# 87003697/DynamiCrafter

Hardware: AMD Instinct MI355X
Metric: frames/sec (and denoising-step ms), 16f@576x1024, DDIM 50 (higher is better)
Workload: dtype bf16; 1 GPU; inference_1024_v1.0.yaml: 1 clip/GPU, 16 frames, latent 72x128, DDIM 50 uniform_trailing eta=1, CFG 7.5 batched (cond+uncond), guidance_rescale 0.7, v-param+ZTSNR+dynamic rescale, hipGraph-captured step; clips_per_gpu=1, parallelism=dp1 over 1 distinct clips (no data-path collective), conditioning=local (1 rank), outputs_finite=True

## Files before the change

### dynamicrafter_amd/_hip.py

```python
import ctypes as C
import os
import threading

_HERE = os.path.dirname(os.path.abspath(__file__))
LIB_PATH = os.environ.get("DC_HIP_LIB") or os.path.join(_HERE, "csrc", "libdcrafter_hip.so")

DC_GEMM_OUT_F32 = 1
DC_GEMM_GEGLU = 2
DC_GEMM_GELU = 4


class DcGemmParams(C.Structure):
    _fields_ = [
        ("A", C.c_void_p), ("W", C.c_void_p), ("C", C.c_void_p), ("bias", C.c_void_p),
        ("rowvec", C.c_void_p), ("residual", C.c_void_p),
        ("lda", C.c_int), ("ldc", C.c_int), ("ldr", C.c_int), ("rowvec_ld", C.c_int),
        ("rows_per_vec", C.c_int),
        ("M", C.c_int), ("N", C.c_int), ("K", C.c_int), ("n_pad", C.c_int),
        ("mode", C.c_int), ("Cin", C.c_int),
        ("IH", C.c_int), ("IW", C.c_int), ("OH", C.c_int), ("OW", C.c_int),
        ("stride", C.c_int), ("pad", C.c_int), ("ups", C.c_int),
        ("T", C.c_int), ("HW", C.c_int),
        ("flags", C.c_int), ("alpha", C.c_float),
        ("workspace", C.c_void_p), ("workspace_bytes", C.c_longlong),
    ]


class DcDdimParams(C.Structure):
    _fields_ = [
        ("a_t", C.c_void_p), ("a_prev", C.c_void_p), ("sigma_t", C.c_void_p), ("sqrt_one_minus_at", C.c_void_p),
        ("sqrt_acp_t", C.c_void_p), ("sqrt_1macp_t", C.c_void_p), ("scale_ratio", C.c_void_p),
        ("step_index", C.c_void_p),
        ("index", C.c_int), ("v_param", C.c_int),
        ("cfg_scale", C.c_float), ("cfg_img", C.c_float), ("guidance_rescale", C.c_float),
        ("temperature", C.c_float),
        ("e_nchw", C.c_int), ("noise_step_stride", C.c_int64),
    ]


class DcDpmParams(C.Structure):
    _fields_ = [
        ("A", C.c_void_p), ("alpha_t", C.c_void_p), ("alpha_p_r", C.c_void_p), ("k", C.c_void_p), ("N", C.c_void_p),
        ("sqrt_one_minus_at", C.c_void_p), ("sqrt_acp_t", C.c_void_p), ("sqrt_1macp_t", C.c_void_p),
        ("scale_ratio", C.c_void_p), ("step_index", C.c_void_p),
        ("index", C.c_int), ("v_param", C.c_int),
        ("cfg_scale", C.c_float), ("cfg_img", C.c_float), ("guidance_rescale", C.c_float),
        ("temperature", C.c_float),
        ("e_nchw", C.c_int), ("noise_step_stride", C.c_int64), ("x0_hist", C.c_void_p),
    ]


class DcSdsParams(C.Structure):
    _fields_ = [
        ("c1", C.c_void_p), ("c2", C.c_void_p), ("w", C.c_void_p), ("step_size", C.c_void_p), ("bc2_sqrt", C.c_void_p),
        ("step_index", C.c_void_p), ("index", C.c_int), ("weight_type", C.c_int), ("x0_param", C.c_int),
        ("e_nchw", C.c_int), ("cfg_scale", C.c_float), ("guidance_rescale", C.c_float),
        ("beta2", C.c_float), ("eps", C.c_float), ("one_minus_beta1", C.c_float), ("one_minus_beta2", C.c_float),
        ("decay", C.c_float), ("grad_scale", C.c_float), ("noise_step_stride", C.c_int64), ("loss", C.c_void_p),
    ]


_P, _I, _F, _L = C.c_void_p, C.c_int, C.c_float, C.c_int64
SIGNATURES = {
    "dc_gemm_conv": (_I, [C.POINTER(DcGemmParams), _P]),
    "dc_gemm_workspace_bytes": (_L, []),
    "dc_gemm_last_variant": (C.c_char_p, []),
    "dc_gemm_set_plan": (_I, [_I]),
    "dc_groupnorm": (_I, [_P, _I, _P, _I, _P, _P, _I, _I, _I, _I, _F, _I, _P, _P]),
    "dc_groupnorm_workspace_bytes": (_L, [_I, _I, _I]),
    "dc_layernorm": (_I, [_P, _I, _P, _I, _P, _P, _I, _I, _F, _P]),
    "dc_flash_attn_d64": (_I, [_P, _P, _P, _P, _I, _I, _I, _I, _I, _I, _I, _I, _L, _L, _F, _I, _F, _P]),
    "dc_ff_geglu_fused320": (_I, [_P, _I, _P, _P, _F, _P, _P, _P, _P, _P, _I, _P, _I, _I, _P]),
    "dc_ff_geglu_proj_fused320": (_I, [_P, _I, _P, _P, _F, _P, _P, _P, _P, _P, _P, _P, _I, _P, _I, _I, _P]),
    "dc_ln_linear": (_I, [_P, _I, _I, _P, _P, _F, _P, _P, _P, _I, _I, _I, _P]),
    "dc_ln_qkv_temporal_attn320": (_I, [_P, _I, _P, _P, _F, _P, _P, _I, _I, _I, _I, _F, _P]),
    "dc_ln_qkv_temporal_attn640": (_I, [_P, _I, _P, _P, _F, _P, _P, _I, _I, _I, _I, _F, _P]),
    "dc_gn_silu_tconv3": (_I, [_P, _I, _I, _P, _P, _P, _I, _P, _P, _P, _I, _P, _I, _I, _I, _I, _I, _P]),
    "dc_groupnorm_stats": (_I, [_P, _I, _I, _I, _I, _I, _F, _P, _P, _P]),
    "dc_gn_linear": (_I, [_P, _I, _I, _P, _P, _P, _I, _I, _P, _P, _P, _I, _I, _I, _P]),
    "dc_flash_attn_set_mode": (_I, [_I, _F]),
    "dc_linear_residual": (_I, [_P, _I, _I, _P, _P, _P, _I, _P, _I, _I, _I, _P]),
    "dc_cross_attn_dual_d64": (_I, [_P, _P, _P, _P, _P, _P, _I, _I, _I, _I, _I, _I, _I, _I, _L, _L, _F, _F, _P]),
    "dc_temporal_attn_d64": (_I, [_P, _I, _P, _I, _I, _I, _I, _I, _F, _P]),
    "dc_gemv_small": (_I, [_P, _I, _P, _P, _P, _I, _I, _I, _I, _I, _I, _I, _P]),
    "dc_timestep_embedding": (_I, [_P, _P, _I, _P, _I, _I, _F, _P]),
    "dc_pack_latent": (_I, [_P, _P, _P, _I, _I, _I, _I, _I, _I, _I, _P]),
    "dc_pack_latent_windows": (_I, [_P, _P, _P, _P, _P] + [_I] * 13 + [_P]),
    "dc_window_merge": (_I, [_P, _I, _P, _I, _P, _P, _P] + [_I] * 12 + [_P]),
    "dc_nchw_to_rows": (_I, [_P, _P, _I, _I, _I, _I, _F, _P]),
    "dc_rows_to_nchw": (_I, [_P, _I, _I, _P, _I, _I, _I, _F, _P]),
    "dc_im2col3x3_c8": (_I, [_P, _I, _P, _I, _I, _I, _I, _P]),
    "dc_copy2d": (_I, [_P, _I, _P, _I, _I, _I, _P]),
    "dc_build_context": (_I, [_P, _P, _I, _I, _I, _I, _I, _P]),
    "dc_softmax_rows": (_I, [_P, _I, _P, _I, _I, _I, _P]),
    "dc_transpose": (_I, [_P, _I, _P, _I, _I, _I, _P]),
    "dc_add_rows": (_I, [_P, _I, _P, _I, _P, _I, _I, _I, _P]),
    "dc_vae_sample": (_I, [_P, _I, _P, _P, _I, _I, _I, _F, _P]),
    "dc_ddim_step": (_I, [C.POINTER(DcDdimParams), _P, _P, _P, _I, _P, _P, _P, _P, _I, _I, _I, _P, _P]),
    "dc_dpmpp_step": (_I, [C.POINTER(DcDpmParams), _P, _P, _P, _I, _P, _P, _P, _P, _I, _I, _I, _P, _P]),
    "dc_sds_noise": (_I, [C.POINTER(DcSdsParams), _P, _P, _P, _I, _L, _P]),
    "dc_sds_step": (_I, [C.POINTER(DcSdsParams), _P, _P, _I, _P, _P, _P, _P, _I, _I, _I, _P, _P]),
    "dc_attn_small": (_I, [_P, _P, _P, _P, _I, _I, _I, _I, _I, _I, _I, _I, _I, _F, _I, _P]),
    "dc_attn_small_lds_bytes": (_L, [_I, _I]),
    "dc_clip_preprocess": (_I, [_P, _P, _P, _P, _I, _I, _I, _I, _I, _I, _I, C.POINTER(_F), C.POINTER(_F), _P]),
    "dc_patchify": (_I, [_P, _P, _I, _I, _I, _I, _I, _I, _P]),
    "dc_embed_tokens": (_I, [_P, _P, _P, _P, _I, _I, _I, _I, _P]),
    "dc_frames_to_u8": (_I, [_P, _P, _I, _I, _I, _I, _I, _P]),
    "dc_jpeg_dct_quant": (_I, [_P, _P, _P, _I, _I, _I, _P]),
    "dc_jpeg_entropy": (_I, [_P, _P, _P, _I, _I, _I, _I, _L, _P]),
    "dc_jpeg_pack": (_I, [_P, _P, _P, _P, _P, _I, _I, _L, _L, _P]),
    "dc_prep_resize_h": (_I, [_P, _P, _P, _P, _P] + [_I] * 8 + [_P]),
    "dc_prep_finish": (_I, [_P, _P, _P, _P, _P] + [_I] * 15 + [_P]),
    "dc_mask_blend": (_I, [_P, _P, _P, _P, _P, _P, _P, _I, _L, _L, _I, _P]),
    "dc_advance_counter": (_I, [_P, _P]),
    "dc_stream_create": (_I, [C.POINTER(_P)]),
    "dc_stream_destroy": (_I, [_P]),
    "dc_stream_sync": (_I, [_P]),
    "dc_graph_begin_capture": (_I, [_P]),
    "dc_graph_end_capture": (_I, [_P, C.POINTER(_P)]),
    "dc_graph_launch": (_I, [_P, _P]),
    "dc_graph_destroy": (_I, [_P]),
    "dc_event_create": (_I, [C.POINTER(_P)]),
    "dc_event_record": (_I, [_P, _P]),
    "dc_event_elapsed_ms": (_I, [_P, _P, C.POINTER(_F)]),
    "dc_event_destroy": (_I, [_P]),
    "dc_error_word_read": (_I, [C.POINTER(C.c_int), _I]),
    "dc_version": (C.c_char_p, []),
}

_lib = None
_lock = threading.Lock()


def lib():
    global _lib
    if _lib is not None:
        return _lib
    with _lock:
        if _lib is None:
            if not os.path.exists(LIB_PATH):
                raise RuntimeError(
                    f"{LIB_PATH} not found: build it with dynamicrafter_amd/csrc/build.sh "
                    "(or __graft_entry__.build()); the HIP extension is mandatory, there is no fallback")
            import torch
            l = C.CDLL(LIB_PATH)
            for name, (res, args) in SIGNATURES.items():
                fn = getattr(l, name)
                fn.restype = res
                fn.argtypes = args
            _lib = l
    return _lib


ERROR_WORD_BITS = {1: "gemm_pipe320x16_kernel: LDS counter wait timed out",
                   2: "flash_attn_d64_pipe_kernel: K/V ring counter wait timed out",
                   4: "gemm_pp_kernel: LDS counter wait timed out"}


def check_error_word(what="", reset=True):
    w = C.c_int(0)
    check(lib().dc_error_word_read(C.byref(w), 1 if reset else 0), "dc_error_word_read")
    if w.value:
        names = [v for k, v in ERROR_WORD_BITS.items() if w.value & k] or [f"unknown bits {w.value:#x}"]
        raise RuntimeError(f"HIP kernels reported a failed wait ({what or 'error word'} = {w.value:#x}): " + "; ".join(names)
                           + " - results since the last check are NOT valid")


def check(code, what):
    if code != 0:
        raise RuntimeError(f"{what} failed with code {code}"
                           + (" (DC_ERR_SHAPE)" if code == -1 else " (DC_ERR_ARG)" if code == -2 else " (hipError_t)"))
```

### dynamicrafter_amd/csrc/dc_common.h

```cpp
#pragma once
#include <hip/hip_runtime.h>
#include <stdint.h>
#include <atomic>

typedef uint16_t bf16_t;

typedef __attribute__((ext_vector_type(8))) short bf16x8_t;
typedef __attribute__((ext_vector_type(4))) short bf16x4_t;
typedef __attribute__((ext_vector_type(16))) float f32x16_t;
typedef __attribute__((ext_vector_type(4))) float f32x4_t;
typedef __attribute__((ext_vector_type(4))) unsigned int u32x4_t;

#define DC_WAVE 64

__device__ __forceinline__ float bf2f(bf16_t v) {
    return __uint_as_float(((uint32_t)v) << 16);
}

typedef __attribute__((ext_vector_type(2))) float f32x2_t;
typedef __attribute__((ext_vector_type(2))) __bf16 bf16x2_hw_t;

__device__ __forceinline__ uint32_t pack_bf2(float lo, float hi) {
    const f32x2_t v = {lo, hi};
    return __builtin_bit_cast(uint32_t, __builtin_convertvector(v, bf16x2_hw_t));
}

__device__ __forceinline__ bf16_t f2bf(float f) { return (bf16_t)(pack_bf2(f, 0.f) & 0xffffu); }

__device__ __forceinline__ void unpack_bf8(const uint4& v, float* f) {
    f[0] = __uint_as_float(v.x << 16); f[1] = __uint_as_float(v.x & 0xffff0000u);
    f[2] = __uint_as_float(v.y << 16); f[3] = __uint_as_float(v.y & 0xffff0000u);
    f[4] = __uint_as_float(v.z << 16); f[5] = __uint_as_float(v.z & 0xffff0000u);
    f[6] = __uint_as_float(v.w << 16); f[7] = __uint_as_float(v.w & 0xffff0000u);
}

__device__ __forceinline__ uint4 pack_bf8(const float* f) {
    uint4 v;
    v.x = pack_bf2(f[0], f[1]); v.y = pack_bf2(f[2], f[3]);
    v.z = pack_bf2(f[4], f[5]); v.w = pack_bf2(f[6], f[7]);
    return v;
}

__device__ __forceinline__ float silu_f(float x) {
    return x * __builtin_amdgcn_rcpf(1.0f + __builtin_amdgcn_exp2f(-1.4426950408889634f * x));
}

__device__ __forceinline__ float erf_as_f(float x) {
    const float ax = fabsf(x);
    const float t = __builtin_amdgcn_rcpf(fmaf(0.3275911f, ax, 1.0f));
    float p = fmaf(1.061405429f, t, -1.453152027f);
    p = fmaf(p, t, 1.421413741f);
    p = fmaf(p, t, -0.284496736f);
    p = fmaf(p, t, 0.254829592f);
    p *= t;
    const float e = __builtin_amdgcn_exp2f(-ax * ax * 1.4426950408889634f);
    const float r = fmaf(-p, e, 1.0f);
    return copysignf(r, x);
}
__device__ __forceinline__ float gelu_erf_f(float x) { return 0.5f * x * (1.0f + erf_as_f(x * 0.70710678118654752f)); }

__device__ __forceinline__ float phi_poly_f(float x) {
    const float xc = __builtin_amdgcn_fmed3f(x, -4.0f, 4.0f);
    const float t = xc * xc;
    float q = fmaf(2.258878772920525e-08f, t, -1.5888579127931735e-06f);
    q = fmaf(q, t, 4.776452260557562e-05f);
    q = fmaf(q, t, -0.0008121939026750624f);
    q = fmaf(q, t, 0.008763724006712437f);
    q = fmaf(q, t, -0.06455449014902115f);
    q = fmaf(q, t, 0.3978703022003174f);
    return fmaf(xc, q, 0.5f);
}
__device__ __forceinline__ float gelu_phi_f(float x) { return x * phi_poly_f(x); }
#ifdef DC_GELU_ERF
#define DC_GELU(x) gelu_erf_f(x)
#else
#define DC_GELU(x) gelu_phi_f(x)
#endif

__device__ __forceinline__ float wave_sum(float v) {
#pragma unroll
    for (int o = 32; o > 0; o >>= 1) v += __shfl_xor(v, o, 64);
    return v;
}
__device__ __forceinline__ float wave_max(float v) {
#pragma unroll
    for (int o = 32; o > 0; o >>= 1) v = fmaxf(v, __shfl_xor(v, o, 64));
    return v;
}

__device__ __forceinline__ int xcd_remap(int bid, int nwg) {
    const int q = nwg >> 3, r = nwg & 7;
    const int xcd = bid & 7, idx = bid >> 3;
    const int base = (xcd < r) ? xcd * (q + 1) : r * (q + 1) + (xcd - r) * q;
    return base + idx;
}

void dc_note_variant(const char* name);

int dc_gemm_plan_now();

int dc_flash_pipe_launch(const bf16_t* q, const bf16_t* k, const bf16_t* v, bf16_t* o, int ldq, int ldk, int ldv, int ldo,
                         int batch, int heads, int Lq, int Lk, int64_t q_bstride, int64_t kv_bstride, float c,
                         hipStream_t stream);

int* dc_error_word_device();
#define DC_ERRW_GEMM_PIPE 1
#define DC_ERRW_FLASH_RING 2
#define DC_ERRW_GEMM_PP 4

struct DcLdsOnce {
    std::atomic<unsigned long long> done{0};
    int ensure(const void* fn, int bytes) {
        int dev = 0;
        hipError_t e = hipGetDevice(&dev);
        if (e != hipSuccess) return (int)e;
        const bool tracked = dev >= 0 && dev < 64;
        if (tracked && (done.load(std::memory_order_acquire) >> dev & 1ull)) return 0;
        e = hipFuncSetAttribute(fn, hipFuncAttributeMaxDynamicSharedMemorySize, bytes);
        if (e != hipSuccess) return (int)e;
        if (tracked) done.fetch_or(1ull << dev, std::memory_order_release);
        return 0;
    }
};

#define DC_CHECK_LAUNCH() do { hipError_t e__ = hipGetLastError(); if (e__ != hipSuccess) return (int)e__; } while (0)
```

### dynamicrafter_amd/csrc/gemm_conv.hip

```cpp
#include "dc_common.h"
#include "dcrafter_hip.h"
#include "lds_stage.h"
#include <stdlib.h>

namespace {

constexpr int BM = 128;
constexpr int BK = 64;
constexpr int NTHREADS = 256;

template <int BN, bool GEGLU, int MODE>
__global__ __launch_bounds__(NTHREADS) void gemm_conv_kernel(const DcGemmParams p) {
    constexpr int NB = BN / 64;
    constexpr int BNOUT = GEGLU ? BN / 2 : BN;
    constexpr int A_BYTES = BM * BK * 2;
    constexpr int B_BYTES = BN * BK * 2;
    constexpr int STAGE = A_BYTES + B_BYTES;
    constexpr int B_ITERS = BN / 32;
    extern __shared__ __attribute__((aligned(16))) char smem[];

    const int tid = threadIdx.x;
    const int lane = tid & 63;
    const int wave = tid >> 6;
    const int wm = wave >> 1, wn = wave & 1;
// ... 373 lines not shown
            const int pc = tid + 256 * i;
            *reinterpret_cast<u32x4_t*>(wst + nc_off(pc >> 3, pc & 7)) = wreg[i];
        }
    };

    const int nslices = p.Cin / 64;
    w_fetch(0, 0);
#pragma unroll 1
    for (int sl = 0; sl < nslices; ++sl) {
        if (sl > 0) __syncthreads();
        for (int g = wave; g < NC_GROUPS; g += 4) {
            const int px = g * 8 + (lane >> 3), ch = (lane & 7) ^ (px & 7);
            const int wy = px / NC_WIN_W, wx = px - wy * NC_WIN_W;
            const int iy = ty0 + wy - 1, ix = tx0 + wx - 1;
            const bool in = px < NC_WIN && iy >= 0 && iy < p.IH && ix >= 0 && ix < p.IW;
            const uint16_t* src = in ? fbase + ((size_t)iy * p.IW + ix) * p.lda + sl * 64 + ch * 8
                                     : reinterpret_cast<const uint16_t*>(g_zero_chunk);
            lds_dma16(src, lds_base + g * 1024);
        }
        w_store();
        wait_vmcnt<0>();
        __syncthreads();
#pragma unroll 1
        for (int t = 0; t < 9; ++t) {
            if (t + 1 < 9) w_fetch(sl, t + 1);
            else if (sl + 1 < nslices) w_fetch(sl + 1, 0);
            const int dy = t / 3, dx = t - 3 * dy;
#pragma unroll
            for (int ks = 0; ks < 2; ++ks) {
                bf16x8_t xb[NC_TW / 16];
#pragma unroll
                for (int b = 0; b < NC_TW / 16; ++b) {
                    const int px = (wave + dy) * NC_WIN_W + 16 * b + lj + dx;
                    xb[b] = *reinterpret_cast<const bf16x8_t*>(win + nc_off(px, ks * 4 + lq));
                }
#pragma unroll
                for (int c = 0; c < WC_CB; ++c) {
                    const bf16x8_t wa = *reinterpret_cast<const bf16x8_t*>(wst + nc_off(c * 16 + lj, ks * 4 + lq));
#pragma unroll
                    for (int b = 0; b < NC_TW / 16; ++b)
                        acc[b][c] = __builtin_amdgcn_mfma_f32_16x16x32_bf16(wa, xb[b], acc[b][c], 0, 0, 0);
                }
            }
            if (t + 1 < 9) {
                __syncthreads();
                w_store();
                __syncthreads();
            }
        }
    }
    __syncthreads();
    const int oy = ty0 + wave;
    if (oy >= p.IH) return;
    char* const patch = wsm + wave * 8192;
    uint16_t* const cbase = reinterpret_cast<uint16_t*>(p.C);
    const int rpx = lane >> 3, rch = lane & 7;
    const size_t row0 = ((size_t)frame * p.IH + oy) * p.IW + tx0;
#pragma unroll
    for (int hf = 0; hf < 2; ++hf) {
        u32x4_t rres[8];
        if (p.residual) {
#pragma unroll
            for (int it = 0; it < 8; ++it) {
                int px = it * 8 + rpx;
                if (tx0 + px >= p.IW) px = 0;
                rres[it] = *reinterpret_cast<const u32x4_t*>(p.residual + (row0 + px) * p.ldr + hf * 64 + rch * 8);
            }
        }
#pragma unroll
        for (int b = 0; b < NC_TW / 16; ++b)
#pragma unroll
            for (int c4 = 0; c4 < 4; ++c4) {
                const int c = hf * 4 + c4;
                float4 v = make_float4(acc[b][c][0], acc[b][c][1], acc[b][c][2], acc[b][c][3]);
                if (p.bias) {
                    const float4 bv = *reinterpret_cast<const float4*>(p.bias + 16 * c + 4 * lq);
                    v.x += bv.x; v.y += bv.y; v.z += bv.z; v.w += bv.w;
                }
                uint2 pk;
                pk.x = pack_bf2(v.x, v.y); pk.y = pack_bf2(v.z, v.w);
                const int px = 16 * b + lj;
                *reinterpret_cast<uint2*>(patch + nc_off(px, 2 * c4 + (lq >> 1)) + (lq & 1) * 8) = pk;
            }
#pragma unroll
        for (int it = 0; it < 8; ++it) {
            const int px = it * 8 + rpx;
            u32x4_t d = *reinterpret_cast<const u32x4_t*>(patch + nc_off(px, rch));
            if (p.residual) {
#pragma unroll
                for (int e = 0; e < 4; ++e)
                    d[e] = pack_bf2(__uint_as_float(d[e] << 16) + __uint_as_float(rres[it][e] << 16),
                                    __uint_as_float(d[e] & 0xffff0000u) + __uint_as_float(rres[it][e] & 0xffff0000u));
            }
            if (tx0 + px < p.IW) *reinterpret_cast<u32x4_t*>(cbase + (row0 + px) * p.ldc + hf * 64 + rch * 8) = d;
        }
    }
}

inline bool window128_conv_ok(const DcGemmParams& p) {
    if ((dc_gemm_plan_now() & 256) || p.mode != 1 || (p.N != WC_N && p.N != 2 * WC_N) || p.stride != 1 || p.pad != 1 || p.ups) return false;
    if (p.OH != p.IH || p.OW != p.IW || p.Cin % 64 != 0 || p.K != 9 * p.Cin || p.n_pad < p.N) return false;
    if (p.rowvec || p.flags || p.alpha != 1.0f) return false;
    if (p.M % (p.IH * p.IW) != 0 || ((uintptr_t)p.A % 16) != 0 || ((uintptr_t)p.W % 16) != 0 || ((uintptr_t)p.C % 8) != 0) return false;
    if (p.ldc % 8 != 0 || ((uintptr_t)p.C % 16) != 0 || (p.residual && (p.ldr % 8 != 0 || ((uintptr_t)p.residual % 16) != 0))) return false;
    const long long tiles = (long long)(p.M / (p.IH * p.IW)) * ((p.IW + NC_TW - 1) / NC_TW) * ((p.IH + NC_TH - 1) / NC_TH);
    return tiles >= 1024;
}

int launch_window128_conv(const DcGemmParams& p, hipStream_t stream) {
    static DcLdsOnce lds_once;
    if (const int e = lds_once.ensure(reinterpret_cast<const void*>(&conv3x3_window128_kernel), WC_LDS)) return e;
    const int tiles_x = (p.IW + NC_TW - 1) / NC_TW, tiles_y = (p.IH + NC_TH - 1) / NC_TH;
    const long long grid = (long long)(p.M / (p.IH * p.IW)) * tiles_x * tiles_y;
    if (grid <= 0 || grid > 0x7fffffffll) return DC_ERR_SHAPE;
    dc_note_variant(p.N == WC_N ? "conv3x3_window128_kernel" : "conv3x3_window128_kernel x2");
    for (int h = 0; h < p.N / WC_N; ++h) {
        DcGemmParams q = p;
        q.W = p.W + (size_t)h * WC_N * p.K;
        if (p.bias) q.bias = p.bias + h * WC_N;
        q.C = reinterpret_cast<uint16_t*>(p.C) + h * WC_N;
        if (p.residual) q.residual = p.residual + h * WC_N;
        q.N = WC_N;
        hipLaunchKernelGGL(conv3x3_window128_kernel, dim3((unsigned)grid), dim3(256), WC_LDS, stream, q, tiles_x, tiles_y);
        DC_CHECK_LAUNCH();
    }
    return 0;
}

inline bool narrow_conv_ok(const DcGemmParams& p) {
    if ((dc_gemm_plan_now() & 128) || p.mode != 1 || p.N > 16 || p.N % 4 != 0 || p.stride != 1 || p.pad != 1 || p.ups) return false;
    if (p.OH != p.IH || p.OW != p.IW || p.Cin % 64 != 0 || p.K != 9 * p.Cin) return false;
    if (p.residual || p.rowvec || (p.flags & ~DC_GEMM_OUT_F32)) return false;
    if (p.M % (p.IH * p.IW) != 0 || ((uintptr_t)p.A % 16) != 0 || ((uintptr_t)p.W % 16) != 0) return false;
    if ((p.flags & DC_GEMM_OUT_F32) ? ((uintptr_t)p.C % 16 != 0) : (((uintptr_t)p.C % 8) != 0)) return false;
    return true;
}

int launch_narrow_conv(const DcGemmParams& p, hipStream_t stream) {
    const int tiles_x = (p.IW + NC_TW - 1) / NC_TW, tiles_y = (p.IH + NC_TH - 1) / NC_TH;
    const long long grid = (long long)(p.M / (p.IH * p.IW)) * tiles_x * tiles_y;
    if (grid <= 0 || grid > 0x7fffffffll) return DC_ERR_SHAPE;
    dc_note_variant("conv3x3_narrow_kernel");
    if (p.flags & DC_GEMM_OUT_F32)
        hipLaunchKernelGGL(conv3x3_narrow_kernel<true>, dim3((unsigned)grid), dim3(256), 0, stream, p, tiles_x, tiles_y);
    else
        hipLaunchKernelGGL(conv3x3_narrow_kernel<false>, dim3((unsigned)grid), dim3(256), 0, stream, p, tiles_x, tiles_y);
    DC_CHECK_LAUNCH();
    return 0;
}

}

int dc_gemm_conv_glds_try(const DcGemmParams& p, hipStream_t stream);

static bool glds_enabled() {
    static int v = -1;
    if (v < 0) {
        const char* e = getenv("DC_GEMM_GLDS");
        v = (e && e[0] == '0') ? 0 : 1;
    }
    return v == 1;
}

static thread_local const char* g_last_variant = "none";
void dc_note_variant(const char* name) { g_last_variant = name; }
extern "C" const char* dc_gemm_last_variant(void) { return g_last_variant; }

extern "C" int64_t dc_gemm_workspace_bytes(void) {
    return (int64_t)8 * 40 * 256 * 320 * 4;
}

extern "C" int dc_gemm_conv(const DcGemmParams* pp, void* stream_) {
    const DcGemmParams& p = *pp;
    hipStream_t stream = (hipStream_t)stream_;
    if (p.M <= 0 || p.N <= 0 || p.K <= 0) return DC_ERR_SHAPE;
    if (p.K % BK != 0 || p.N % 4 != 0 || p.lda % 8 != 0 || p.ldc % 4 != 0) return DC_ERR_SHAPE;
    if (p.mode != 0 && (p.Cin % BK != 0)) return DC_ERR_SHAPE;
    if (p.mode == 1 && p.K != 9 * p.Cin) return DC_ERR_SHAPE;
    if (p.mode == 2 && p.K != 3 * p.Cin) return DC_ERR_SHAPE;
    if (p.residual && (p.ldr % 4 != 0)) return DC_ERR_SHAPE;
    const bool geglu = (p.flags & DC_GEMM_GEGLU) != 0;
    if (geglu && ((p.N / 2) % 64 != 0 || p.n_pad < p.N)) return DC_ERR_SHAPE;
    if (p.n_pad < (p.N + 127) / 128 * 128) return DC_ERR_SHAPE;
    if (narrow_conv_ok(p)) return launch_narrow_conv(p, stream);
    if (window128_conv_ok(p)) return launch_window128_conv(p, stream);
    if (glds_enabled()) {
        const int r = dc_gemm_conv_glds_try(p, stream);
        if (r != -100) return r;
    }
    if (geglu) return launch<128, true>(p, stream);
    const int t128 = (p.N + 127) / 128 * 128;
    const bool use64 = (p.N <= 64) || ((float)t128 / (float)p.N > 1.15f);
    if (use64) {
        if (p.n_pad < (p.N + 63) / 64 * 64) return DC_ERR_SHAPE;
        return launch<64, false>(p, stream);
    }
    if (p.n_pad < t128) return DC_ERR_SHAPE;
    return launch<128, false>(p, stream);
}
```

### dynamicrafter_amd/csrc/gemm_conv_glds.hip

```cpp
#include "dc_common.h"
#include "dcrafter_hip.h"
#include "lds_stage.h"
#include <stdint.h>
#include <stdlib.h>
#include <type_traits>
#include <utility>

namespace {

constexpr int GBM = 256;
constexpr int GBK = 64;
constexpr int GNT = 512;

struct GemmSplit {
    float* partial;
    int splits;
    int tile_begin;
    int tile_count;
    int* err;
    int whole;
};

template <int BN, bool GEGLU, int MODE, int GSTAGES>
__global__ __launch_bounds__(GNT) void gemm_conv_glds_kernel(const DcGemmParams p, const GemmSplit sp) {
// ... 651 lines not shown
                    int brow;
                    if (GEGLU) brow = (nb < NBX ? 0 : BN / 2) + wn * (BN / 4) + (nb % NBX) * 32;
                    else brow = wn * (32 * NB) + nb * 32;
                    wf[nb] = *reinterpret_cast<const bf16x8_t*>(sb + lds_off128(brow + fr, kk * 2 + fh));
                }
#pragma unroll
                for (int mb = 0; mb < 2; ++mb)
#pragma unroll
                    for (int nb = 0; nb < NB; ++nb)
                        acc[mb][nb] = __builtin_amdgcn_mfma_f32_32x32x16_bf16(wf[nb], xf[mb], acc[mb][nb], 0, 0, 0);
            }
        }
        if (++stage >= GSTAGES) stage = 0;
        if (++c_kt >= nk) {
            if constexpr (RES_RING) {
#pragma unroll
                for (int j = 0; j < NB; ++j) {
                    ++g;
                    const int younger_r = total - 1 - g;
                    if (GSTAGES >= 3 && younger_r >= 1) {
                        if (j + 1 < NB) wait_vmcnt<A_IT>(); else wait_vmcnt<LOADS>();
                    } else {
                        wait_vmcnt<0>();
                    }
                    __builtin_amdgcn_s_barrier();
                    asm volatile("" ::: "memory");
                    if (g + GSTAGES - 1 < total) {
#pragma unroll
                        for (int kk = 0; kk < GBK / 16; ++kk) issue_next_part(kk);
                    }
                    const char* sr = smem + stage * STAGE;
                    int lane_r = lane;
                    asm volatile("" : "+v"(lane_r));
                    const int fr_r = lane_r & 31, fh_r = lane_r >> 5;
#pragma unroll
                    for (int i = 0; i < 2; ++i) {
                        const int e1 = fr_r - 16 * i - 8 * fh_r;
                        bf16x8_t idf;
#pragma unroll
                        for (int e = 0; e < 8; ++e) idf[e] = (e == e1) ? (short)0x3F80 : (short)0;
#pragma unroll
                        for (int mb = 0; mb < 2; ++mb) {
                            const bf16x8_t xr = *reinterpret_cast<const bf16x8_t*>(
                                sr + lds_off128(wm * 64 + mb * 32 + fr_r, (wn * 2 + i) * 2 + fh_r));
                            acc[mb][j] = __builtin_amdgcn_mfma_f32_32x32x16_bf16(idf, xr, acc[mb][j], 0, 0, 0);
                        }
                    }
                    if (++stage >= GSTAGES) stage = 0;
                }
            }
            c_kt = 0;
            const int logical = xcd_remap((int)blockIdx.x + c_tile * G, ntiles);
            ++c_tile;
            int tn, tmi;
            persist_tile(logical, tiles_m, tiles_n, tile_group, tmi, tn);
            const int m0 = tmi * GBM, n0 = tn * BNOUT;
            persist_epilogue<BN, GEGLU, EPI>(acc, p, m0, n0, n_out, wm, wn, lane, smem + GSTAGES * STAGE + wave * 2048);
            zero_acc();
        }
    }
}

template <int BN, bool GEGLU, int EPI, int MODE, int ST_FORCE>
int launch_persist_epi_st(const DcGemmParams& p, hipStream_t stream, int grid);

template <int BN, bool GEGLU, int EPI, int MODE>
int launch_persist_epi(const DcGemmParams& p, hipStream_t stream, int grid) {
    static const int st = [] { const char* e = getenv("DC_GEMM_STAGES"); return e ? atoi(e) : 0; }();
    if constexpr (BN <= 128 && MODE == 0 && !GEGLU) { if (st == 2) return launch_persist_epi_st<BN, GEGLU, EPI, MODE, 2>(p, stream, grid); }
    return launch_persist_epi_st<BN, GEGLU, EPI, MODE, 0>(p, stream, grid);
}

template <int BN, bool GEGLU, int EPI, int MODE, int ST_FORCE>
int launch_persist_epi_st(const DcGemmParams& p, hipStream_t stream, int grid) {
    constexpr int ST = ST_FORCE ? ST_FORCE : ((BN <= 128) ? 3 : 2);
    constexpr size_t lds = (size_t)ST * (GBM * GBK * 2 + BN * GBK * 2) + 8 * 2048;
    static_assert(lds <= 163840, "LDS budget");
    static DcLdsOnce lds_once;
    if (const int e = lds_once.ensure(reinterpret_cast<const void*>(&gemm_persist_kernel<BN, GEGLU, ST, EPI, MODE>), (int)lds)) return e;
    dc_note_variant(GEGLU ? (BN == 256 ? "gemm_persist_kernel<256,geglu>" : "gemm_persist_kernel<128,geglu>")
                    : MODE == 1 ? "gemm_persist_kernel<320,conv>" : MODE == 2 ? "gemm_persist_kernel<320,tconv>"
                    : BN == 320 ? (EPI == 1 || EPI == 3 ? "gemm_persist_kernel<320,residual>" : "gemm_persist_kernel<320>")
                    : BN == 128 ? "gemm_persist_kernel<128>" : "gemm_persist_kernel<64>");
    static const int group = [] { const char* e = getenv("DC_GEMM_GROUP"); return e ? atoi(e) : 8; }();
    hipLaunchKernelGGL((gemm_persist_kernel<BN, GEGLU, ST, EPI, MODE>), dim3(grid), dim3(GNT), lds, stream, p,
                       (group == 2 || group == 4 || group == 8 || group == 16) ? group : 1);
    DC_CHECK_LAUNCH();
    return 0;
}

inline bool ring_residual_ok(const DcGemmParams& p) {
    static const int on = [] { const char* e = getenv("DC_GEMM_RING_RESIDUAL"); return e ? atoi(e) : 1; }();
    return on && p.residual && !(p.flags & (DC_GEMM_GELU | DC_GEMM_GEGLU | DC_GEMM_OUT_F32)) && p.alpha == 1.0f &&
           (p.N % 64 == 0) && (p.ldr % 8 == 0) && ((uintptr_t)p.residual % 16 == 0);
}

template <int BN, bool GEGLU>
int launch_persist(const DcGemmParams& p, hipStream_t stream, int grid) {
    if (p.flags & DC_GEMM_OUT_F32) {
        if constexpr (GEGLU) return DC_ERR_ARG;
        else return launch_persist_epi<BN, GEGLU, 2, 0>(p, stream, grid);
    }
    if (p.residual) {
        if constexpr (!GEGLU) { if (ring_residual_ok(p) && p.N % BN == 0) return launch_persist_epi<BN, GEGLU, 3, 0>(p, stream, grid); }
        return launch_persist_epi<BN, GEGLU, 1, 0>(p, stream, grid);
    }
    return launch_persist_epi<BN, GEGLU, 0, 0>(p, stream, grid);
}

int launch_persist_conv320(const DcGemmParams& p, hipStream_t stream) {
    const bool ring = ring_residual_ok(p);
    if (p.mode == 1) return p.residual ? (ring ? launch_persist_epi<320, false, 3, 1>(p, stream, 256)
                                               : launch_persist_epi<320, false, 1, 1>(p, stream, 256))
                                       : launch_persist_epi<320, false, 0, 1>(p, stream, 256);
    return p.residual ? (ring ? launch_persist_epi<320, false, 3, 2>(p, stream, 256)
                              : launch_persist_epi<320, false, 1, 2>(p, stream, 256))
                      : launch_persist_epi<320, false, 0, 2>(p, stream, 256);
}

template <int BN, bool GEGLU, int MODE, int GSTAGES>
int launch_glds(const DcGemmParams& p, hipStream_t stream) {
    constexpr int BNOUT = GEGLU ? BN / 2 : BN;
    const int n_out = GEGLU ? p.N / 2 : p.N;
    const int tiles_n = (n_out + BNOUT - 1) / BNOUT;
    const int tiles_m = (p.M + GBM - 1) / GBM;
    constexpr size_t lds = (size_t)GSTAGES * (GBM * GBK * 2 + BN * GBK * 2);
    static DcLdsOnce lds_once;
    if (const int e = lds_once.ensure(reinterpret_cast<const void*>(&gemm_conv_glds_kernel<BN, GEGLU, MODE, GSTAGES>), (int)lds)) return e;
    GemmSplit sp;
    sp.partial = nullptr; sp.splits = 1; sp.tile_begin = 0; sp.tile_count = tiles_m * tiles_n; sp.err = nullptr; sp.whole = 0;
    dc_note_variant(GEGLU ? "gemm_conv_glds_kernel<geglu>"
                    : BN == 320 ? (MODE == 0 ? "gemm_conv_glds_kernel<320>" : MODE == 2 ? "gemm_conv_glds_kernel<320,tconv>" : "gemm_conv_glds_kernel<320,conv>")
                    : BN == 256 ? (MODE == 0 ? "gemm_conv_glds_kernel<256>" : MODE == 2 ? "gemm_conv_glds_kernel<256,tconv>" : "gemm_conv_glds_kernel<256,conv>")
                    : (MODE == 0 ? "gemm_conv_glds_kernel<128>" : MODE == 2 ? "gemm_conv_glds_kernel<128,tconv>" : "gemm_conv_glds_kernel<128,conv>"));
    hipLaunchKernelGGL((gemm_conv_glds_kernel<BN, GEGLU, MODE, GSTAGES>), dim3(tiles_m * tiles_n), dim3(GNT), lds, stream, p, sp);
    DC_CHECK_LAUNCH();
    return 0;
}

constexpr int PLAN_DEFAULT = 3 | 16;
constexpr int PLAN_MASK = 3 | 16 | 32 | 64 | 128 | 256;
inline bool plan_valid(int plan) { return plan >= 0 && plan <= 511 && !(plan & 4); }
std::atomic<int> g_gemm_plan{[] {
    const char* e = getenv("DC_GEMM_PLAN");
    const int v = e ? atoi(e) : PLAN_DEFAULT;
    return plan_valid(v) ? (v & PLAN_MASK) : PLAN_DEFAULT;
}()};
inline int pipe_min_k() { static const int v = [] { const char* e = getenv("DC_PIPE_MIN_K"); return e ? atoi(e) : 1920; }(); return v; }

template <int MODE, int EPI>
int launch_pipe_shape(const DcGemmParams& p, hipStream_t stream, GemmSplit sp, int gx, int gy) {
    sp.err = dc_error_word_device();
    if (!sp.err) return DC_ERR_ARG;
    return launch_pipe320x16<MODE, EPI>(p, stream, sp, gx, gy);
}

inline bool pipe_ok(const DcGemmParams& p, int plan) {
    if (!(plan & 3) || (!(plan & 2) && p.mode != 1)) return false;
    if (p.mode != 1 && p.K < pipe_min_k()) return false;
    if (p.flags & (DC_GEMM_GEGLU | DC_GEMM_OUT_F32)) return false;
    if (p.ups && !(p.mode == 1 && p.ups == 1 && p.stride == 1 && p.pad == 1 && p.OH == 2 * p.IH && p.OW == 2 * p.IW)) return false;
    if (p.N % 320 != 0 || p.n_pad < p.N || p.K % 64 != 0 || p.lda % 8 != 0 || ((uintptr_t)p.A % 16) != 0) return false;
    if (p.ldc % 8 != 0 || ((uintptr_t)p.C % 16) != 0 || (long long)p.M * p.ldc >= (1ll << 31)) return false;
    if (p.residual && (p.ldr % 8 != 0 || ((uintptr_t)p.residual % 16) != 0 || (long long)p.M * p.ldr >= (1ll << 31))) return false;
    long long rows = p.M, extra = 0;
    if (p.mode == 1) { if (p.Cin % 64 != 0 || p.K != 9 * p.Cin) return false; rows = (long long)(p.M / (p.OH * p.OW) + 1) * p.IH * p.IW; extra = 2ll * p.IW + 2; }
    else if (p.mode == 2) { if (p.Cin % 64 != 0 || p.K != 3 * p.Cin) return false; extra = 2ll * p.HW; }
    else if (p.mode != 0) return false;
    if ((rows + extra) * p.lda * 2 >= (1ll << 31)) return false;
    if (320ll * p.K * 2 >= (1ll << 31)) return false;
    return true;
}

int launch_pipe_whole(const DcGemmParams& p, hipStream_t stream) {
    const int ntiles = ((p.M + GBM - 1) / GBM) * (p.N / 320);
    GemmSplit sp;
    sp.partial = nullptr; sp.splits = 1; sp.tile_begin = 0; sp.tile_count = ntiles; sp.err = nullptr; sp.whole = 0;
    dc_note_variant(p.mode == 0 ? "gemm_pipe320x16_kernel" : p.mode == 2 ? "gemm_pipe320x16_kernel<tconv>"
                    : p.ups ? "gemm_pipe320x16_kernel<conv,ups>" : "gemm_pipe320x16_kernel<conv>");
    if (p.mode == 0) return p.residual ? launch_pipe_shape<0, 1>(p, stream, sp, ntiles, 1) : launch_pipe_shape<0, 0>(p, stream, sp, ntiles, 1);
    if (p.mode == 1 && p.ups) return p.residual ? launch_pipe_shape<3, 1>(p, stream, sp, ntiles, 1) : launch_pipe_shape<3, 0>(p, stream, sp, ntiles, 1);
    if (p.mode == 1) return p.residual ? launch_pipe_shape<1, 1>(p, stream, sp, ntiles, 1) : launch_pipe_shape<1, 0>(p, stream, sp, ntiles, 1);
    return p.residual ? launch_pipe_shape<2, 1>(p, stream, sp, ntiles, 1) : launch_pipe_shape<2, 0>(p, stream, sp, ntiles, 1);
}

template <int MODE, int BN = 320>
int launch_glds320_split(const DcGemmParams& p, hipStream_t stream, int ntiles, int full, int splits, bool use_pipe, bool merged) {
    constexpr int GSTAGES = 2;
    constexpr size_t lds = (size_t)GSTAGES * (GBM * GBK * 2 + BN * GBK * 2);
    static DcLdsOnce lds_once;
    if (const int e = lds_once.ensure(reinterpret_cast<const void*>(&gemm_conv_glds_kernel<BN, false, MODE, GSTAGES>), (int)lds)) return e;
    if constexpr (BN == 320) {
        if (use_pipe) {
            dc_note_variant(MODE == 0 ? "gemm_pipe320x16_kernel+splitk" : MODE == 2 ? "gemm_pipe320x16_kernel<tconv>+splitk"
                            : MODE == 3 ? "gemm_pipe320x16_kernel<conv,ups>+splitk" : "gemm_pipe320x16_kernel<conv>+splitk");
            GemmSplit sp;
            sp.err = nullptr; sp.whole = 0;
            if (full > 0 && merged && full % 8 == 0) {
                sp.partial = reinterpret_cast<float*>(p.workspace); sp.splits = splits; sp.tile_begin = full; sp.tile_count = ntiles - full;
                sp.whole = full;
                const int gx = full + sp.tile_count * splits;
                if (const int e = p.residual ? launch_pipe_shape<MODE, 1>(p, stream, sp, gx, 1) : launch_pipe_shape<MODE, 0>(p, stream, sp, gx, 1)) return e;
                sp.whole = 0;
            } else {
                if (full > 0) {
                    sp.partial = nullptr; sp.splits = 1; sp.tile_begin = 0; sp.tile_count = full;
                    if (const int e = p.residual ? launch_pipe_shape<MODE, 1>(p, stream, sp, full, 1) : launch_pipe_shape<MODE, 0>(p, stream, sp, full, 1)) return e;
                }
                sp.partial = reinterpret_cast<float*>(p.workspace); sp.splits = splits; sp.tile_begin = full; sp.tile_count = ntiles - full;
                if (const int e = launch_pipe_shape<MODE, 0>(p, stream, sp, sp.tile_count, splits)) return e;
            }
            hipLaunchKernelGGL((splitk_reduce_kernel<BN>), dim3((GBM * (BN / 4) + 255) / 256, sp.tile_count), dim3(256), 0, stream, p, sp);
            DC_CHECK_LAUNCH();
            return 0;
        }
    }
    if constexpr (BN == 320)
        dc_note_variant(MODE == 0 ? "gemm_conv_glds_kernel<320>+splitk" : MODE == 2 ? "gemm_conv_glds_kernel<320,tconv>+splitk" : "gemm_conv_glds_kernel<320,conv>+splitk");
    else
        dc_note_variant(MODE == 0 ? "gemm_conv_glds_kernel<256>+splitk" : MODE == 2 ? "gemm_conv_glds_kernel<256,tconv>+splitk" : "gemm_conv_glds_kernel<256,conv>+splitk");
    GemmSplit sp;
    sp.err = nullptr; sp.whole = 0;
    if (full > 0) {
        sp.partial = nullptr; sp.splits = 1; sp.tile_begin = 0; sp.tile_count = full;
        hipLaunchKernelGGL((gemm_conv_glds_kernel<BN, false, MODE, GSTAGES>), dim3(full), dim3(GNT), lds, stream, p, sp);
        DC_CHECK_LAUNCH();
    }
    sp.partial = reinterpret_cast<float*>(p.workspace); sp.splits = splits; sp.tile_begin = full; sp.tile_count = ntiles - full;
    hipLaunchKernelGGL((gemm_conv_glds_kernel<BN, false, MODE, GSTAGES>), dim3(sp.tile_count, splits), dim3(GNT), lds, stream, p, sp);
    DC_CHECK_LAUNCH();
    hipLaunchKernelGGL((splitk_reduce_kernel<BN>), dim3((GBM * (BN / 4) + 255) / 256, sp.tile_count), dim3(256), 0, stream, p, sp);
    DC_CHECK_LAUNCH();
    return 0;
}

template <int BN, int GSTAGES>
int launch_glds_mode(const DcGemmParams& p, hipStream_t stream) {
    if (p.mode == 0) return launch_glds<BN, false, 0, GSTAGES>(p, stream);
    if (p.mode == 1) return p.ups ? launch_glds<BN, false, 3, GSTAGES>(p, stream) : launch_glds<BN, false, 1, GSTAGES>(p, stream);
    return launch_glds<BN, false, 2, GSTAGES>(p, stream);
}

inline int persist_max_k() {
    static const int v = [] { const char* e = getenv("DC_GEMM_PERSIST_MAXK"); return e ? atoi(e) : 2560; }();
    return v;
}

inline float wave_eff(int wgs) { return (float)wgs / (float)(((wgs + 255) / 256) * 256); }

}

int dc_gemm_conv_glds_try(const DcGemmParams& p, hipStream_t stream) {
    const bool geglu = (p.flags & DC_GEMM_GEGLU) != 0;
    const int n_out = geglu ? p.N / 2 : p.N;
    const int tiles_m = (p.M + GBM - 1) / GBM;
    static const int force = [] { const char* e = getenv("DC_GEMM_TILE"); return e ? atoi(e) : 0; }();
    static const int persist = [] { const char* e = getenv("DC_GEMM_PERSIST"); return e ? atoi(e) : 1; }();
    if (geglu && p.mode != 0) return DC_ERR_ARG;
    const bool out_f32 = (p.flags & DC_GEMM_OUT_F32) != 0;
    const bool epi16 = out_f32 || ((n_out % 8 == 0) && (p.ldc % 8 == 0) && ((long long)p.M * p.ldc < (1ll << 31)) &&
                                   ((long long)p.M * p.ldr < (1ll << 31)) && ((uintptr_t)p.C % 16 == 0) &&
                                   (!p.residual || ((p.ldr % 8 == 0) && ((uintptr_t)p.residual % 16 == 0))));
    const int plan = g_gemm_plan.load(std::memory_order_relaxed);
    const bool use_pipe = pipe_ok(p, plan);
    const bool prefer_pipe = (force == 0) && use_pipe;
    if (persist && force == 0 && p.mode == 0 && epi16 && p.K <= persist_max_k() && !prefer_pipe) {
        static const int wide = [] { const char* e = getenv("DC_GEMM_PERSIST_WIDE"); return e ? atoi(e) : 1; }();
        if (geglu && (plan & 16) && ((plan & 32) || p.K <= 640) && pp_ok(p) && tiles_m * (n_out / 64) >= 1024) return launch_pp(p, stream);
        if (geglu) {
            if (wide && n_out % 128 == 0 && tiles_m * (n_out / 128) >= 512) return launch_persist<256, true>(p, stream, 256);
            const int nt = tiles_m * (n_out / 64);
            if (nt >= 512) return launch_persist<128, true>(p, stream, 256);
        } else {
            if (wide && p.N % 320 == 0 && p.n_pad >= p.N && tiles_m * (p.N / 320) >= 512)
                return launch_persist<320, false>(p, stream, 256);
            const int t128n = (p.N + 127) / 128;
            const float waste = (float)(t128n * 128) / (float)p.N;
            if (waste <= 1.15f && tiles_m * t128n >= 512) return launch_persist<128, false>(p, stream, 256);
            const int t64n = (p.N + 63) / 64;
            if (waste > 1.15f && tiles_m * t64n >= 512) return launch_persist<64, false>(p, stream, 256);
        }
    }
    static const int persist_conv_maxk = [] { const char* e = getenv("DC_GEMM_PERSIST_CONV_MAXK"); return e ? atoi(e) : 2880; }();
    if (persist && force == 0 && !prefer_pipe && !geglu && !out_f32 && epi16 && (p.mode == 2 || (p.mode == 1 && !p.ups)) &&
        p.N % 320 == 0 && p.n_pad >= p.N && tiles_m * (p.N / 320) >= (p.mode == 1 ? 1024 : 512) && p.K <= persist_conv_maxk)
        return launch_persist_conv320(p, stream);
    if (geglu) {
        const int w256 = (n_out % 128 == 0 && p.n_pad >= p.N) ? tiles_m * (n_out / 128) : 0;
        const int w128 = tiles_m * (n_out / 64);
        if ((force == 256 || (force == 0 && w256 >= 512 && wave_eff(w256) > 0.8f)) && w256 > 0)
            return launch_glds<256, true, 0, 2>(p, stream);
        if (w128 < 384) return -100;
        return launch_glds<128, true, 0, 3>(p, stream);
    }
    const int t128 = (p.N + 127) / 128;
    const bool n320 = (p.N % 320 == 0) && (p.n_pad >= p.N);
    const int w320 = n320 ? tiles_m * (p.N / 320) : 0;
    const int w128 = tiles_m * t128;
    const float waste128 = (float)(t128 * 128) / (float)p.N;
    const bool pipe_conv = use_pipe && p.mode == 1 && force == 0;
    float s320 = n320 ? (pipe_conv ? 1.4f : 1.25f) * wave_eff(w320) : 0.f;
    float s128 = wave_eff(w128) / waste128;
    if (w320 < (pipe_conv ? 128 : 200)) s320 = 0.f;
    if (w128 < 384) s128 = 0.f;
    static const int splitk = [] { const char* e = getenv("DC_GEMM_SPLITK"); return e ? atoi(e) : 1; }();
    if (splitk && force == 0 && n320 && p.workspace && p.n_pad >= p.N) {
        const int nk = p.K / GBK;
        int full = 0, splits = 0;
        if (w320 < 200 && w320 >= 8) {
            splits = 256 / w320;
            if (splits > 12) splits = 12;
            while (splits > 2 && nk / splits < 12) --splits;
        } else if (w320 > 256 && w320 <= 1280 && (w320 % 256) != 0 && (w320 % 256) <= 128) {
            full = (w320 / 256) * 256;
            splits = 256 / (w320 - full);
            if (splits > 8) splits = 8;
            while (splits > 2 && nk / splits < 8) --splits;
        }
        const size_t need = (size_t)splits * (size_t)(w320 - full) * GBM * 320 * sizeof(float);
        if (splits >= 2 && nk / splits >= (full ? 8 : 12) && need <= (size_t)p.workspace_bytes) {
            const bool merged = !(plan & 64);
            if (p.mode == 0) return launch_glds320_split<0>(p, stream, w320, full, splits, use_pipe, merged);
            if (p.mode == 1) return p.ups ? launch_glds320_split<3>(p, stream, w320, full, splits, use_pipe, merged)
                                          : launch_glds320_split<1>(p, stream, w320, full, splits, use_pipe, merged);
            return launch_glds320_split<2>(p, stream, w320, full, splits, use_pipe, merged);
        }
    }
    static const int splitk256 = [] { const char* e = getenv("DC_GEMM_SPLITK256"); return e ? atoi(e) : 1; }();
    if (splitk && splitk256 && force == 0 && !n320 && !out_f32 && p.workspace && p.N % 256 == 0 && p.n_pad >= p.N && (p.mode != 1 || !p.ups)) {
        const int w256s = tiles_m * (p.N / 256), nk = p.K / GBK;
        if (w256s > 256 && w256s <= 1280 && (w256s % 256) != 0 && (w256s % 256) <= 128) {
            const int full = (w256s / 256) * 256;
            int splits = 256 / (w256s - full);
            if (splits > 8) splits = 8;
            while (splits > 2 && nk / splits < 8) --splits;
            const size_t need = (size_t)splits * (size_t)(w256s - full) * GBM * 256 * sizeof(float);
            if (splits >= 2 && nk / splits >= 8 && need <= (size_t)p.workspace_bytes) {
                if (p.mode == 0) return launch_glds320_split<0, 256>(p, stream, w256s, full, splits, false, false);
                if (p.mode == 1) return launch_glds320_split<1, 256>(p, stream, w256s, full, splits, false, false);
                return launch_glds320_split<2, 256>(p, stream, w256s, full, splits, false, false);
            }
        }
    }
    if (force == 320 && n320) return use_pipe ? launch_pipe_whole(p, stream) : launch_glds_mode<320, 2>(p, stream);
    if (force == 128 && w128 > 0 && waste128 <= 1.15f) return launch_glds_mode<128, 3>(p, stream);
    if (force == 1) return -100;
    const int w256 = (!n320 && p.N % 256 == 0 && p.n_pad >= p.N) ? tiles_m * (p.N / 256) : 0;
    if ((force == 256 || force == 0) && w256 >= 200 && 1.2f * wave_eff(w256) >= s128) return launch_glds_mode<256, 2>(p, stream);
    if (s320 > 0.f && s320 >= s128) return use_pipe ? launch_pipe_whole(p, stream) : launch_glds_mode<320, 2>(p, stream);
    if (s128 > 0.f && waste128 <= 1.15f) return launch_glds_mode<128, 3>(p, stream);
    return -100;
}

int dc_gemm_plan_now() { return g_gemm_plan.load(std::memory_order_relaxed); }

extern "C" int dc_gemm_set_plan(int plan) {
    if (!plan_valid(plan)) return DC_ERR_ARG;
    return g_gemm_plan.exchange(plan & PLAN_MASK, std::memory_order_relaxed);
}
```

### dynamicrafter_amd/csrc/gemm_pipe16.h

```cpp
#pragma once

typedef __attribute__((ext_vector_type(4))) float gp_f32x4_t;

#define GP16_MFMA_A(d, w, x) asm volatile("v_mfma_f32_16x16x32_bf16 %0, %1, %2, %0" : "+a"(d) : "v"(w), "v"(x))
#define GP16_MFMA_V(d, w, x) asm volatile("v_mfma_f32_16x16x32_bf16 %0, %1, %2, %0" : "+v"(d) : "v"(w), "v"(x))

__device__ __forceinline__ void gp16_settle(gp_f32x4_t (&acc)[4][20]) {
#pragma unroll
    for (int rb = 0; rb < 4; ++rb)
        asm volatile("s_nop 7\n\ts_nop 7"
                     : "+a"(acc[rb][0]), "+a"(acc[rb][1]), "+a"(acc[rb][2]), "+a"(acc[rb][3]), "+a"(acc[rb][4]), "+a"(acc[rb][5]),
                       "+a"(acc[rb][6]), "+a"(acc[rb][7]), "+a"(acc[rb][8]), "+a"(acc[rb][9]), "+a"(acc[rb][10]), "+a"(acc[rb][11]),
                       "+a"(acc[rb][12]), "+a"(acc[rb][13]), "+a"(acc[rb][14]), "+a"(acc[rb][15]), "+v"(acc[rb][16]), "+v"(acc[rb][17]),
                       "+v"(acc[rb][18]), "+v"(acc[rb][19]));
    asm volatile("s_nop 7\n\ts_nop 7" ::: "memory");
}

template <int MODE, int EPI>
__global__ __launch_bounds__(256, 1) __attribute__((amdgpu_waves_per_eu(1, 1)))
void gemm_pipe320x16_kernel(const DcGemmParams p, const GemmSplit sp) {
    extern __shared__ __attribute__((aligned(16))) char smem[];
    const int tid = threadIdx.x, lane = tid & 63;
    const int wave = __builtin_amdgcn_readfirstlane(tid >> 6);
    const int lr = lane & 15, lq = lane >> 4;

    const int tiles_n = p.N / 320;
    int bx = blockIdx.x, by = blockIdx.y, tile_begin = sp.tile_begin, tile_count = sp.tile_count, nsplit = sp.splits;
    float* partial = sp.partial;
    if (sp.whole > 0) {
        if (bx < sp.whole) { tile_begin = 0; tile_count = sp.whole; nsplit = 1; partial = nullptr; by = 0; }
        else { bx -= sp.whole; by = bx / tile_count; bx -= by * tile_count; }
    }
    const int swz = tile_begin + xcd_remap(bx, tile_count);
    const int tile_n = swz % tiles_n;
    const int tile_m = swz / tiles_n;
    const int m0 = tile_m * GBM;
    const int n0 = tile_n * 320;

    const int nk_all = p.K / GBK;
    const int kt_lo = (int)(((long long)by * nk_all) / nsplit);
    const int kt_hi = (int)(((long long)(by + 1) * nk_all) / nsplit);
    const int nk = kt_hi - kt_lo;

    lds_int_t* const cnt_landed = (lds_int_t*)(smem + GP_CNT);
    lds_int_t* const cnt_freed = cnt_landed + 1;
    if (tid < 2) cnt_landed[tid] = 0;
    __syncthreads();
    int gave_up = 0;

    const unsigned lda2 = (unsigned)p.lda * 2u;
    unsigned rowoff[4];
    int mask[4];
    long long bias = 0;
    if (MODE == 1) bias = (long long)(p.pad * p.IW + p.pad) * lda2;
    if (MODE == 2) bias = (long long)p.HW * lda2;
    if (MODE == 3) bias = (long long)(p.IW + 1) * lda2;
#ifdef GP_DBG_QUAD_ROWS
    const int lr_a = lr & ~3, lq_a = lane & 3;
#else
    const int lr_a = lr, lq_a = lq;
#endif
#pragma unroll
    for (int rb = 0; rb < 4; ++rb) {
        const int m = m0 + wave * 64 + rb * 16 + lr_a;
        const bool ok = m < p.M;
        const int mm = ok ? m : 0;
        if (MODE == 0) {
            rowoff[rb] = (unsigned)mm * lda2 + lq_a * 16;
            mask[rb] = ok ? 1 : 0;
        } else if (MODE == 1) {
            const int ohw = p.OH * p.OW;
            const int n = mm / ohw;
            const int rem = mm - n * ohw;
            const int oy = rem / p.OW;
            const int ox = rem - oy * p.OW;
            const int iy0 = oy * p.stride - p.pad, ix0 = ox * p.stride - p.pad;
            int mk = 0;
#pragma unroll
            for (int t = 0; t < 9; ++t) {
                const int iy = iy0 + t / 3, ix = ix0 + t % 3;
                if (ok && iy >= 0 && iy < p.IH && ix >= 0 && ix < p.IW) mk |= 1 << t;
            }
            mask[rb] = mk;
            rowoff[rb] = (unsigned)(((n * p.IH + iy0 + p.pad) * p.IW + ix0 + p.pad)) * lda2 + lq_a * 16;
        } else if (MODE == 3) {
            const int ohw = p.OH * p.OW;
            const int n = mm / ohw;
            const int rem = mm - n * ohw;
            const int oy = rem / p.OW;
            const int ox = rem - oy * p.OW;
            int mk = 0;
#pragma unroll
            for (int t = 0; t < 9; ++t) {
                const int uy = oy + t / 3 - 1, ux = ox + t % 3 - 1;
                if (ok && uy >= 0 && uy < p.OH && ux >= 0 && ux < p.OW) mk |= 1 << t;
            }
            mask[rb] = mk | ((oy & 1) << 9) | ((ox & 1) << 10);
            rowoff[rb] = (unsigned)(((n * p.IH + (oy >> 1) + 1) * p.IW + (ox >> 1) + 1)) * lda2 + lq_a * 16;
        } else {
            const int frame = (mm / p.HW) % p.T;
            int mk = 0;
#pragma unroll
            for (int t = 0; t < 3; ++t) {
                const int tt = frame + t - 1;
                if (ok && tt >= 0 && tt < p.T) mk |= 1 << t;
            }
            mask[rb] = mk;
            rowoff[rb] = (unsigned)mm * lda2 + lq_a * 16;
        }
    }
    gp_i32x4_t ars;
    {
        const unsigned long long ab = (unsigned long long)(uintptr_t)p.A - (unsigned long long)bias;
        ars[0] = __builtin_amdgcn_readfirstlane((int)(unsigned)ab);
        ars[1] = __builtin_amdgcn_readfirstlane((int)(unsigned)((ab >> 32) & 0xffffu));
        ars[2] = 0x7fffffff;
        ars[3] = 0x00020000;
    }
    auto a_tile = [&](int kt, unsigned (&vo)[4], int& soff) __attribute__((always_inline)) {
        int tap = 0;
        if (MODE == 0) {
            soff = kt * 128;
        } else if (MODE == 1) {
            const int cs = kt / 9;
            tap = kt - cs * 9;
            const int dy = tap / 3, dx = tap - dy * 3;
            soff = (dy * p.IW + dx) * (int)lda2 + cs * 128;
        } else if (MODE == 3) {
            const int cs = kt / 9;
            tap = kt - cs * 9;
            const int dy = tap / 3, dx = tap - dy * 3;
            soff = cs * 128;
            const int y0 = dy == 0 ? -p.IW * (int)lda2 : 0, y1 = dy == 2 ? p.IW * (int)lda2 : 0;
            const int x0 = dx == 0 ? -(int)lda2 : 0, x1 = dx == 2 ? (int)lda2 : 0;
#pragma unroll
            for (int rb = 0; rb < 4; ++rb) {
                const unsigned o = rowoff[rb] + (unsigned)(((mask[rb] >> 9) & 1) ? y1 : y0) + (unsigned)(((mask[rb] >> 10) & 1) ? x1 : x0);
                vo[rb] = ((mask[rb] >> tap) & 1) ? o : 0x80000000u;
            }
            return;
        } else {
            const int cs = kt / 3;
            tap = kt - cs * 3;
            soff = tap * p.HW * (int)lda2 + cs * 128;
        }
#pragma unroll
        for (int rb = 0; rb < 4; ++rb) vo[rb] = ((mask[rb] >> tap) & 1) ? rowoff[rb] : 0x80000000u;
    };

    const unsigned lds_base = (unsigned)(uintptr_t)((const lds_char_t*)smem);
    unsigned voffB[10];
#pragma unroll
    for (int j = 0; j < 10; ++j) {
        const int row = (j * 4 + wave) * 8 + (lane >> 3);
        voffB[j] = (unsigned)row * (unsigned)p.K * 2u + (unsigned)(((lane & 7) ^ (((wave & 1) * 4 + (lane >> 4)) & 7)) << 4);
        asm volatile("" : "+v"(voffB[j]));
    }
    auto w_src = [&](int kt) __attribute__((always_inline)) -> unsigned long long {
        return (unsigned long long)(uintptr_t)p.W + ((unsigned long long)n0 * p.K + (unsigned long long)kt * 64) * 2ull;
    };

    unsigned bofs[3][2];
#pragma unroll
    for (int st = 0; st < 3; ++st)
#pragma unroll
        for (int s = 0; s < 2; ++s) {
            bofs[st][s] = lds_base + st * GP_STAGE + lr * 128 + (((4 * s + lq) ^ ((lr >> 1) & 7)) << 4);
            asm volatile("" : "+v"(bofs[st][s]));
        }
    bf16x8_t Bf[5];
    auto rd_b = [&](int slot, unsigned addr, int cb) __attribute__((always_inline)) {
        Bf[slot] = *(lds_vfrag_t*)((const lds_char_t*)(uintptr_t)addr + cb * 2048);
    };

    u32x4_t A[3][4][2];
    gp_f32x4_t acc[4][20];
#pragma unroll
    for (int i = 0; i < 4; ++i)
#pragma unroll
        for (int j = 0; j < 20; ++j)
#pragma unroll
            for (int r = 0; r < 4; ++r) acc[i][j][r] = 0.f;

    auto clampk = [&](int t) { return kt_lo + (t < nk ? t : nk - 1); };
#pragma unroll
    for (int t = 0; t < 2; ++t) {
        const unsigned long long ws = w_src(clampk(t));
#pragma unroll
        for (int j = 0; j < 10; ++j) lds_dma16_sbase(lds_base + t * GP_STAGE + (j * 4 + wave) * 1024, voffB[j], ws);
        unsigned vo[4];
        int soff;
        a_tile(clampk(t), vo, soff);
#pragma unroll
        for (int i = 0; i < 8; ++i) {
            if ((i >> 2) == 0) GP_LOAD_A_(A[t][i & 3][0], vo[i & 3], ars, soff, "0");
            else GP_LOAD_A_(A[t][i & 3][1], vo[i & 3], ars, soff, "64");
        }
    }
    wait_vmcnt<26>();
    if (lane == 0) __hip_atomic_fetch_add(cnt_landed, 1, __ATOMIC_RELAXED, __HIP_MEMORY_SCOPE_WORKGROUP);
    {
        int seen = *(volatile lds_int_t*)cnt_landed;
        LDS_SPIN(__builtin_amdgcn_readfirstlane(seen) < 4, seen = *(volatile lds_int_t*)cnt_landed);
        asm volatile("" ::: "memory");
    }
#pragma unroll
    for (int f = 0; f < 4; ++f) rd_b(f, bofs[0][0], f);
    gp16_settle(acc);

    int seen_f = 0, seen_l = 0;
    auto tile = [&](auto ST_, int t) __attribute__((always_inline)) {
        constexpr int ST = decltype(ST_)::value, ST1 = (ST + 1) % 3, ST2 = (ST + 2) % 3;
        const int kt2 = clampk(t + 2);
        unsigned vo[4] = {0u, 0u, 0u, 0u};
        int soff = 0;
        unsigned long long ws = 0;
        gp_f32x4_t (&acc1)[4][20] = acc;
        bf16x8_t (&Bf1)[5] = Bf;
        u32x4_t (&A1)[3][4][2] = A;
        for_ic(std::make_integer_sequence<int, 160>{}, [&](auto G_) __attribute__((always_inline)) {
            constexpr int g = decltype(G_)::value;
            gp_f32x4_t (&acc_)[4][20] = acc1;
            bf16x8_t (&Bf_)[5] = Bf1;
            u32x4_t (&A_)[3][4][2] = A1;
            if constexpr (g == 0) {
                wait_vmcnt<18>();
#pragma unroll
                for (int i = 0; i < 8; ++i) asm volatile("" : "+v"(A_[ST][i & 3][i >> 2]));
            }
            if constexpr ((g & 3) == 0) {
                constexpr int F = g / 4 + 4;
                if constexpr (F < 40) rd_b(F % 5, bofs[ST][F / 20], F % 20);
                else rd_b(F % 5, bofs[ST1][0], F - 40);
            } else if constexpr ((g & 3) == 2) {
                if constexpr (g == 2) seen_f = *(volatile lds_int_t*)cnt_freed;
                if constexpr (g == 6) {
                    LDS_SPIN(__builtin_amdgcn_readfirstlane(seen_f) < 4 * t, seen_f = *(volatile lds_int_t*)cnt_freed);
                    asm volatile("" ::: "memory");
                    ws = w_src(kt2);
                }
                if constexpr (g >= 10 && g <= 82 && ((g - 10) & 7) == 0) {
                    constexpr int j = (g - 10) >> 3;
                    lds_dma16_sbase(lds_base + ST2 * GP_STAGE + (j * 4 + wave) * 1024, voffB[j], ws);
                }
                if constexpr (g == 86) {
                    wait_vmcnt<18>();
#ifdef GP_DBG_SKIP_POST
                    if (lane == 0 && !(wave == 3 && t == 1))
#else
                    if (lane == 0)
#endif
                        __hip_atomic_fetch_add(cnt_landed, 1, __ATOMIC_RELAXED, __HIP_MEMORY_SCOPE_WORKGROUP);
                    a_tile(kt2, vo, soff);
                }
                if constexpr (g >= 90 && g <= 146 && ((g - 90) & 7) == 0) {
                    constexpr int i = (g - 90) >> 3;
                    if constexpr ((i >> 2) == 0) GP_LOAD_A_(A_[ST2][i & 3][0], vo[i & 3], ars, soff, "0");
                    else GP_LOAD_A_(A_[ST2][i & 3][1], vo[i & 3], ars, soff, "64");
                }
                if constexpr (g == 118) seen_l = *(volatile lds_int_t*)cnt_landed;
                if constexpr (g == 142) {
                    LDS_SPIN(t + 1 < nk && __builtin_amdgcn_readfirstlane(seen_l) < 4 * (t + 2), seen_l = *(volatile lds_int_t*)cnt_landed);
                    asm volatile("" ::: "memory");
                }
                if constexpr (g == 150) {
                    if (lane == 0) __hip_atomic_fetch_add(cnt_freed, 1, __ATOMIC_RELAXED, __HIP_MEMORY_SCOPE_WORKGROUP);
                }
            }
            constexpr int f = g / 4, rb = g & 3, s = f / 20, cb = f % 20;
            if constexpr (cb < 16) GP16_MFMA_A(acc_[rb][cb], Bf_[f % 5], A_[ST][rb][s]);
            else GP16_MFMA_V(acc_[rb][cb], Bf_[f % 5], A_[ST][rb][s]);
        });
    };
#ifdef GP_STAMPS
    const unsigned long long st_loop0 = __builtin_readcyclecounter();
    const unsigned long long st_real0 = __builtin_amdgcn_s_memrealtime();
#endif
    for (int t = 0; t < nk; t += 3) {
        tile(ic<0>{}, t);
        if (t + 1 >= nk) break;
        tile(ic<1>{}, t + 1);
        if (t + 2 >= nk) break;
        tile(ic<2>{}, t + 2);
    }
    wait_vmcnt<0>();
    gp16_settle(acc);
    if (gave_up && lane == 0) atomicOr(sp.err, DC_ERRW_GEMM_PIPE);
#ifdef GP_STAMPS
    if (lane == 0 && p.workspace && !sp.partial && (size_t)(blockIdx.x * 4 + wave + 1) * 64 <= (size_t)p.workspace_bytes) {
        unsigned long long* out = reinterpret_cast<unsigned long long*>(p.workspace) + (size_t)(blockIdx.x * 4 + wave) * 8;
        out[0] = 0; out[1] = 0; out[2] = 0; out[3] = 0;
        out[4] = __builtin_readcyclecounter() - st_loop0; out[5] = (unsigned long long)nk;
        out[6] = __builtin_amdgcn_s_memrealtime() - st_real0;
    }
#endif

    if (partial) {
        const size_t slot = (size_t)by * tile_count + (size_t)(swz - tile_begin);
        float* const dst = partial + (slot * GBM + wave * 64 + lr) * 320 + 4 * lq;
#pragma unroll
        for (int rb = 0; rb < 4; ++rb)
#pragma unroll
            for (int cb = 0; cb < 20; ++cb)
                *reinterpret_cast<float4*>(dst + (size_t)rb * 16 * 320 + cb * 16) = make_float4(acc[rb][cb][0], acc[rb][cb][1], acc[rb][cb][2], acc[rb][cb][3]);
        return;
    }
    char* const ebuf = smem + GP_RING + wave * 2048;
    int lane_e = lane;
    asm volatile("" : "+v"(lane_e));
    const int er = lane_e & 15, eq = lane_e >> 4;
    const int rrow = lane_e >> 2, rc = lane_e & 3;
    const char* const rbase = reinterpret_cast<const char*>(p.residual);
    char* const cbase = reinterpret_cast<char*>(p.C);
#pragma unroll
    for (int rb = 0; rb < 4; ++rb) {
        const int m_acc = m0 + wave * 64 + rb * 16 + er;
        const float* rv = p.rowvec ? p.rowvec + (size_t)((m_acc < p.M ? m_acc : 0) / p.rows_per_vec) * p.rowvec_ld : nullptr;
        int mr = m0 + wave * 64 + rb * 16 + rrow;
        const bool rok = mr < p.M;
        if (!rok) mr = p.M - 1;
        const unsigned co = ((unsigned)mr * (unsigned)p.ldc + (unsigned)(n0 + rc * 8)) * 2u;
        const unsigned ro = ((unsigned)mr * (unsigned)p.ldr + (unsigned)(n0 + rc * 8)) * 2u;
#pragma unroll
        for (int cp = 0; cp < 10; ++cp) {
            u32x4_t rr;
            if constexpr (EPI == 1) rr = *reinterpret_cast<const u32x4_t*>(rbase + ro + cp * 64);
#pragma unroll
            for (int h = 0; h < 2; ++h) {
                const int cb = 2 * cp + h;
                const int n = n0 + cb * 16 + 4 * eq;
                float4 v = make_float4(acc[rb][cb][0], acc[rb][cb][1], acc[rb][cb][2], acc[rb][cb][3]);
                if (p.bias) {
                    const float4 bv = *reinterpret_cast<const float4*>(p.bias + n);
                    v.x += bv.x; v.y += bv.y; v.z += bv.z; v.w += bv.w;
                }
                if (p.flags & DC_GEMM_GELU) { v.x = DC_GELU(v.x); v.y = DC_GELU(v.y); v.z = DC_GELU(v.z); v.w = DC_GELU(v.w); }
                if (rv) {
                    const float4 r4 = *reinterpret_cast<const float4*>(rv + n);
                    v.x += r4.x; v.y += r4.y; v.z += r4.z; v.w += r4.w;
                }
                if (p.alpha != 1.0f) { v.x *= p.alpha; v.y *= p.alpha; v.z *= p.alpha; v.w *= p.alpha; }
                uint2 pk;
                pk.x = pack_bf2(v.x, v.y);
                pk.y = pack_bf2(v.z, v.w);
                *reinterpret_cast<uint2*>(ebuf + er * 64 + ((((4 * h + eq) ^ (((er >> 1) & 3) << 1))) << 3)) = pk;
            }
            u32x4_t d = *reinterpret_cast<const u32x4_t*>(ebuf + rrow * 64 + ((rc ^ ((rrow >> 1) & 3)) << 4));
            if constexpr (EPI == 1) {
#pragma unroll
                for (int e = 0; e < 4; ++e)
                    d[e] = pack_bf2(__uint_as_float(d[e] << 16) + __uint_as_float(rr[e] << 16),
                                    __uint_as_float(d[e] & 0xffff0000u) + __uint_as_float(rr[e] & 0xffff0000u));
            }
            if (rok) *reinterpret_cast<u32x4_t*>(cbase + co + cp * 64) = d;
            __builtin_amdgcn_sched_barrier(0);
        }
    }
}

template <int MODE, int EPI>
int launch_pipe320x16(const DcGemmParams& p, hipStream_t stream, const GemmSplit& sp, int grid_x, int grid_y) {
    static DcLdsOnce lds_once;
    if (const int e = lds_once.ensure(reinterpret_cast<const void*>(&gemm_pipe320x16_kernel<MODE, EPI>), GP_LDS)) return e;
    hipLaunchKernelGGL((gemm_pipe320x16_kernel<MODE, EPI>), dim3(grid_x, grid_y), dim3(256), GP_LDS, stream, p, sp);
    DC_CHECK_LAUNCH();
    return 0;
}
```

### dynamicrafter_amd/csrc/norms.hip

```cpp
#include "dc_common.h"
#include "dcrafter_hip.h"
#include <stdlib.h>

namespace {

struct GnGeom { int chunks; int rows_per_chunk; };

__host__ __device__ inline GnGeom gn_geom(int n_inst, int rows_per_inst) {
    int chunks = (2048 + n_inst - 1) / n_inst;
    int rpc = (rows_per_inst + chunks - 1) / chunks;
    if (rpc < 64) rpc = 64;
    GnGeom g;
    g.rows_per_chunk = rpc;
    g.chunks = (rows_per_inst + rpc - 1) / rpc;
    return g;
}

__global__ void gn_partial_kernel(const bf16_t* __restrict__ x, int ldx, int C, int groups, int rows_per_inst,
                                  int rows_per_chunk, int chunks, int vecs, int rpp, float2* __restrict__ partial) {
    extern __shared__ float sm[];
    const int inst = blockIdx.y, chunk = blockIdx.x;
    const int v = threadIdx.x % vecs;
    const int ro = threadIdx.x / vecs;
    const int r_begin = chunk * rows_per_chunk;
    int r_end = r_begin + rows_per_chunk;
    if (r_end > rows_per_inst) r_end = rows_per_inst;
    float s[8], ss[8], K[8];
#pragma unroll
    for (int e = 0; e < 8; ++e) { s[e] = 0.f; ss[e] = 0.f; K[e] = 0.f; }
    const bf16_t* base = x + (size_t)inst * rows_per_inst * ldx + v * 8;
    int r = r_begin + ro;
    const int n_t = r < r_end ? (r_end - r + rpp - 1) / rpp : 0;
    bool have_k = false;
    for (; r + 7 * rpp < r_end; r += 8 * rpp) {
        uint4 raw[8];
#pragma unroll
        for (int u = 0; u < 8; ++u) raw[u] = *reinterpret_cast<const uint4*>(base + (size_t)(r + u * rpp) * ldx);
        if (!have_k) { unpack_bf8(raw[0], K); have_k = true; }
#pragma unroll
        for (int u = 0; u < 8; ++u) {
            float f[8];
            unpack_bf8(raw[u], f);
#pragma unroll
            for (int e = 0; e < 8; ++e) { const float d = f[e] - K[e]; s[e] += d; ss[e] += d * d; }
        }
    }
    for (; r < r_end; r += rpp) {
        const uint4 raw = *reinterpret_cast<const uint4*>(base + (size_t)r * ldx);
        float f[8];
        unpack_bf8(raw, f);
        if (!have_k) { unpack_bf8(raw, K); have_k = true; }
#pragma unroll
        for (int e = 0; e < 8; ++e) { const float d = f[e] - K[e]; s[e] += d; ss[e] += d * d; }
    }
    float* sm_s = sm;
    float* sm_q = sm + rpp * C;
    const float inv_n = n_t > 0 ? 1.0f / (float)n_t : 0.f;
#pragma unroll
    for (int e = 0; e < 8; ++e) {
        sm_s[ro * C + v * 8 + e] = K[e] + s[e] * inv_n;
        sm_q[ro * C + v * 8 + e] = ss[e] - s[e] * s[e] * inv_n;
    }
    __syncthreads();
    if ((int)threadIdx.x < groups) {
        const int cpg = C / groups;
        const int g = threadIdx.x;
        float n = 0.f, mean = 0.f, m2 = 0.f;
        for (int rr = 0; rr < rpp; ++rr) {
            const int first = r_begin + rr;
            const float nb = first < r_end ? (float)((r_end - first + rpp - 1) / rpp) : 0.f;
            if (nb == 0.f) continue;
            for (int c = 0; c < cpg; ++c) {
                const float mb = sm_s[rr * C + g * cpg + c], qb = sm_q[rr * C + g * cpg + c];
                const float nn = n + nb;
                const float w = nb * __builtin_amdgcn_rcpf(nn);
                const float delta = mb - mean;
                mean += delta * w;
                m2 += qb + delta * delta * (n * w);
                n = nn;
            }
        }
        partial[((size_t)inst * chunks + chunk) * groups + g] = make_float2(mean, m2);
    }
}

__global__ __launch_bounds__(64) void gn_finalize_kernel(const float2* __restrict__ partial, int chunks, int groups,
                                                         int rows_per_inst, int rows_per_chunk, int cpg, float eps,
                                                         float2* __restrict__ stats) {
    const int g = blockIdx.x, inst = blockIdx.y;
    float n = 0.f, mean = 0.f, m2 = 0.f;
    for (int c = threadIdx.x; c < chunks; c += 64) {
        const float2 p = partial[((size_t)inst * chunks + c) * groups + g];
        int rows = rows_per_inst - c * rows_per_chunk;
        if (rows > rows_per_chunk) rows = rows_per_chunk;
        const float nb = (float)rows * (float)cpg;
        const float nn = n + nb;
        const float w = nb * __builtin_amdgcn_rcpf(nn);
        const float delta = p.x - mean;
        mean += delta * w;
        m2 += p.y + delta * delta * (n * w);
        n = nn;
    }
#pragma unroll
    for (int o = 32; o > 0; o >>= 1) {
        const float nb = __shfl_xor(n, o, 64), mb = __shfl_xor(mean, o, 64), qb = __shfl_xor(m2, o, 64);
        const float nn = n + nb;
        if (nn > 0.f) {
            const float w = nb * __builtin_amdgcn_rcpf(nn);
            const float delta = mb - mean;
            mean += delta * w;
            m2 += qb + delta * delta * (n * w);
            n = nn;
        }
    }
    if (threadIdx.x == 0) {
        float var = m2 / n;
        if (var < 0.f) var = 0.f;
        stats[(size_t)inst * groups + g] = make_float2(mean, rsqrtf(var + eps));
    }
}

template <bool FIN>
__global__ void gn_apply_kernel(const bf16_t* __restrict__ x, int ldx, bf16_t* __restrict__ y, int ldy,
                                const float* __restrict__ gamma, const float* __restrict__ beta, int C, int groups,
                                int rows_per_inst, int rows_per_chunk, int vecs, int rpp, int silu,
                                const float2* __restrict__ stats, int chunks, float eps) {
    const int inst = blockIdx.y, chunk = blockIdx.x;
    __shared__ float2 st_s[64];
    if constexpr (FIN) {
        const int t = threadIdx.x, sub = t & 7;
        const int gpp = (int)blockDim.x >> 3;
        const float cpg = (float)(C / groups);
        for (int g0 = 0; g0 < groups; g0 += gpp) {
            const int g = g0 + (t >> 3);
            float n = 0.f, mean = 0.f, m2 = 0.f;
            if (g < groups) {
                for (int c = sub; c < chunks; c += 8) {
                    const float2 p = stats[((size_t)inst * chunks + c) * groups + g];
                    int rows = rows_per_inst - c * rows_per_chunk;
                    if (rows > rows_per_chunk) rows = rows_per_chunk;
                    const float nb = (float)rows * cpg;
                    const float nn = n + nb;
                    const float w = nb * __builtin_amdgcn_rcpf(nn);
                    const float delta = p.x - mean;
                    mean += delta * w;
                    m2 += p.y + delta * delta * (n * w);
                    n = nn;
                }
            }
#pragma unroll
            for (int o = 1; o < 8; o <<= 1) {
                const float nb = __shfl_xor(n, o, 64), mb = __shfl_xor(mean, o, 64), qb = __shfl_xor(m2, o, 64);
                const float nn = n + nb;
                if (nn > 0.f) {
                    const float lo_n = (sub & o) ? nb : n, lo_m = (sub & o) ? mb : mean, lo_q = (sub & o) ? qb : m2;
                    const float hi_n = (sub & o) ? n : nb, hi_m = (sub & o) ? mean : mb, hi_q = (sub & o) ? m2 : qb;
                    const float w = hi_n * __builtin_amdgcn_rcpf(nn);
                    const float delta = hi_m - lo_m;
                    mean = lo_m + delta * w;
                    m2 = lo_q + hi_q + delta * delta * (lo_n * w);
                    n = nn;
                }
            }
            if (g < groups && sub == 0) {
                float var = m2 / n;
                if (var < 0.f) var = 0.f;
                st_s[g] = make_float2(mean, rsqrtf(var + eps));
            }
        }
        __syncthreads();
    }
    const int v = threadIdx.x % vecs;
    const int ro = threadIdx.x / vecs;
    const int r_begin = chunk * rows_per_chunk;
    int r_end = r_begin + rows_per_chunk;
    if (r_end > rows_per_inst) r_end = rows_per_inst;
    const int cpg = C / groups;
    float sc[8], sh[8];
#pragma unroll
    for (int e = 0; e < 8; ++e) {
        const int c = v * 8 + e;
        const float2 st = FIN ? st_s[c / cpg] : stats[(size_t)inst * groups + c / cpg];
        const float g = gamma[c] * st.y;
        sc[e] = g;
        sh[e] = beta[c] - st.x * g;
    }
    const bf16_t* xb = x + (size_t)inst * rows_per_inst * ldx + v * 8;
    bf16_t* yb = y + (size_t)inst * rows_per_inst * ldy + v * 8;
    int r = r_begin + ro;
    for (; r + 7 * rpp < r_end; r += 8 * rpp) {
        uint4 raw[8];
#pragma unroll
        for (int u = 0; u < 8; ++u) raw[u] = *reinterpret_cast<const uint4*>(xb + (size_t)(r + u * rpp) * ldx);
#pragma unroll
        for (int u = 0; u < 8; ++u) {
            float f[8];
            unpack_bf8(raw[u], f);
#pragma unroll
            for (int e = 0; e < 8; ++e) {
                float t = f[e] * sc[e] + sh[e];
                if (silu) t = silu_f(t);
                f[e] = t;
            }
            *reinterpret_cast<uint4*>(yb + (size_t)(r + u * rpp) * ldy) = pack_bf8(f);
        }
    }
    for (; r < r_end; r += rpp) {
        const uint4 raw = *reinterpret_cast<const uint4*>(xb + (size_t)r * ldx);
        float f[8];
        unpack_bf8(raw, f);
#pragma unroll
        for (int e = 0; e < 8; ++e) {
            float t = f[e] * sc[e] + sh[e];
            if (silu) t = silu_f(t);
            f[e] = t;
        }
        *reinterpret_cast<uint4*>(yb + (size_t)r * ldy) = pack_bf8(f);
    }
}

template <int MAXV>
__global__ __launch_bounds__(256) void layernorm_kernel(const bf16_t* __restrict__ x, int ldx, bf16_t* __restrict__ y,
                                                        int ldy, const float* __restrict__ gamma,
                                                        const float* __restrict__ beta, int rows, int C, float eps) {
    const int lane = threadIdx.x & 63;
    const int wave = threadIdx.x >> 6;
    const int vecs = C >> 3;
    const float invC = 1.0f / (float)C;
    for (int row0 = (blockIdx.x * 4 + wave) * 2; row0 < rows; row0 += gridDim.x * 8) {
        float f[2][MAXV][8];
        float s[2] = {0.f, 0.f};
#pragma unroll
        for (int u = 0; u < 2; ++u) {
            const int row = row0 + u < rows ? row0 + u : rows - 1;
#pragma unroll
            for (int j = 0; j < MAXV; ++j) {
                const int v = lane + 64 * j;
                if (v < vecs) {
                    const uint4 raw = *reinterpret_cast<const uint4*>(x + (size_t)row * ldx + v * 8);
                    unpack_bf8(raw, f[u][j]);
#pragma unroll
                    for (int e = 0; e < 8; ++e) s[u] += f[u][j][e];
                }
            }
        }
#pragma unroll
        for (int u = 0; u < 2; ++u) {
            const int row = row0 + u;
            const float mean = wave_sum(s[u]) * invC;
            float q = 0.f;
#pragma unroll
            for (int j = 0; j < MAXV; ++j) {
                const int v = lane + 64 * j;
                if (v < vecs) {
#pragma unroll
                    for (int e = 0; e < 8; ++e) { const float d = f[u][j][e] - mean; q += d * d; }
                }
            }
            const float rstd = rsqrtf(wave_sum(q) * invC + eps);
            if (row < rows) {
#pragma unroll
                for (int j = 0; j < MAXV; ++j) {
                    const int v = lane + 64 * j;
                    if (v < vecs) {
                        float o[8];
#pragma unroll
                        for (int e = 0; e < 8; ++e) {
                            const int c = v * 8 + e;
                            o[e] = (f[u][j][e] - mean) * rstd * gamma[c] + beta[c];
                        }
                        *reinterpret_cast<uint4*>(y + (size_t)row * ldy + v * 8) = pack_bf8(o);
                    }
                }
            }
        }
    }
}

}

extern "C" int64_t dc_groupnorm_workspace_bytes(int n_inst, int groups, int rows_per_inst) {
    const GnGeom g = gn_geom(n_inst, rows_per_inst);
    return (int64_t)sizeof(float2) * ((int64_t)n_inst * g.chunks * groups + (int64_t)n_inst * groups) + 256;
}

extern "C" int dc_groupnorm(const uint16_t* x, int ldx, uint16_t* y, int ldy, const float* gamma, const float* beta,
                            int C, int groups, int n_inst, int rows_per_inst, float eps, int silu,
                            float* workspace, void* stream_) {
    hipStream_t stream = (hipStream_t)stream_;
    if (!x || !y || !gamma || !beta || !workspace) return DC_ERR_ARG;
    if (C % 8 != 0 || groups <= 0 || groups > 64 || C % groups != 0 || ldx % 8 != 0 || ldy % 8 != 0) return DC_ERR_SHAPE;
    if (n_inst <= 0 || rows_per_inst <= 0) return DC_ERR_SHAPE;
    const int vecs = C / 8;
    if (vecs > 1024) return DC_ERR_SHAPE;
    int rpp = 256 / vecs;
    if (rpp < 1) rpp = 1;
    const int threads = vecs * rpp;
    const GnGeom g = gn_geom(n_inst, rows_per_inst);
    float2* partial = reinterpret_cast<float2*>(workspace);
    float2* stats = partial + (size_t)n_inst * g.chunks * groups;
    const size_t lds = (size_t)2 * rpp * C * sizeof(float);
    if (lds > 64 * 1024) return DC_ERR_SHAPE;
    hipLaunchKernelGGL(gn_partial_kernel, dim3(g.chunks, n_inst), dim3(threads), lds, stream, x, ldx, C, groups,
                       rows_per_inst, g.rows_per_chunk, g.chunks, vecs, rpp, partial);
    DC_CHECK_LAUNCH();
    static const bool fuse_fin = [] { const char* e = getenv("DC_GN_FUSE_FINALIZE"); return !(e && e[0] == '0'); }();
    if (fuse_fin && g.chunks <= 64 && threads % 8 == 0) {
        hipLaunchKernelGGL(gn_apply_kernel<true>, dim3(g.chunks, n_inst), dim3(threads), 0, stream, x, ldx, y, ldy, gamma, beta,
                           C, groups, rows_per_inst, g.rows_per_chunk, vecs, rpp, silu, (const float2*)partial, g.chunks, eps);
        DC_CHECK_LAUNCH();
        return 0;
    }
    hipLaunchKernelGGL(gn_finalize_kernel, dim3(groups, n_inst), dim3(64), 0, stream, partial, g.chunks, groups, rows_per_inst,
                       g.rows_per_chunk, C / groups, eps, stats);
    DC_CHECK_LAUNCH();
    hipLaunchKernelGGL(gn_apply_kernel<false>, dim3(g.chunks, n_inst), dim3(threads), 0, stream, x, ldx, y, ldy, gamma, beta,
                       C, groups, rows_per_inst, g.rows_per_chunk, vecs, rpp, silu, (const float2*)stats, g.chunks, eps);
    DC_CHECK_LAUNCH();
    return 0;
}

extern "C" int dc_groupnorm_stats(const uint16_t* x, int ldx, int C, int groups, int n_inst, int rows_per_inst, float eps,
                                  float* workspace, float* stats_out, void* stream_) {
    hipStream_t stream = (hipStream_t)stream_;
    if (!x || !workspace || !stats_out) return DC_ERR_ARG;
    if (C % 8 != 0 || groups <= 0 || groups > 64 || C % groups != 0 || ldx % 8 != 0) return DC_ERR_SHAPE;
    if (n_inst <= 0 || rows_per_inst <= 0) return DC_ERR_SHAPE;
    const int vecs = C / 8;
    if (vecs > 1024) return DC_ERR_SHAPE;
    int rpp = 256 / vecs;
    if (rpp < 1) rpp = 1;
    const int threads = vecs * rpp;
    const GnGeom g = gn_geom(n_inst, rows_per_inst);
    float2* partial = reinterpret_cast<float2*>(workspace);
    const size_t lds = (size_t)2 * rpp * C * sizeof(float);
    if (lds > 64 * 1024) return DC_ERR_SHAPE;
    hipLaunchKernelGGL(gn_partial_kernel, dim3(g.chunks, n_inst), dim3(threads), lds, stream, x, ldx, C, groups,
                       rows_per_inst, g.rows_per_chunk, g.chunks, vecs, rpp, partial);
    DC_CHECK_LAUNCH();
    hipLaunchKernelGGL(gn_finalize_kernel, dim3(groups, n_inst), dim3(64), 0, stream, partial, g.chunks, groups, rows_per_inst,
                       g.rows_per_chunk, C / groups, eps, reinterpret_cast<float2*>(stats_out));
    DC_CHECK_LAUNCH();
    return 0;
}

extern "C" int dc_layernorm(const uint16_t* x, int ldx, uint16_t* y, int ldy, const float* gamma, const float* beta,
                            int rows, int C, float eps, void* stream_) {
    hipStream_t stream = (hipStream_t)stream_;
    if (!x || !y || !gamma || !beta) return DC_ERR_ARG;
    if (C % 8 != 0 || C > 2048 || ldx % 8 != 0 || ldy % 8 != 0 || rows <= 0) return DC_ERR_SHAPE;
    int grid = (rows + 7) / 8;
    if (grid > 8192) grid = 8192;
    const int vecs = C / 8;
    if (vecs <= 64)
        hipLaunchKernelGGL(layernorm_kernel<1>, dim3(grid), dim3(256), 0, stream, x, ldx, y, ldy, gamma, beta, rows, C, eps);
    else if (vecs <= 128)
        hipLaunchKernelGGL(layernorm_kernel<2>, dim3(grid), dim3(256), 0, stream, x, ldx, y, ldy, gamma, beta, rows, C, eps);
    else
        hipLaunchKernelGGL(layernorm_kernel<4>, dim3(grid), dim3(256), 0, stream, x, ldx, y, ldy, gamma, beta, rows, C, eps);
    DC_CHECK_LAUNCH();
    return 0;
}
```

### dynamicrafter_amd/lvdm/modules/networks/openaimodel3d.py

```python
import math

import torch
import torch.nn as nn

from .... import ops
from ....ops import PackedWeight
from ....param_tree import attach_params

import os

_BF16 = torch.bfloat16
_FF_FUSED = os.environ.get("DC_FF_FUSED", "1") != "0"
_LN_FUSED = os.environ.get("DC_LN_FUSED", "1") != "0"
_LR_FUSED = os.environ.get("DC_LR_FUSED", "1") != "0"
_TA_FUSED = os.environ.get("DC_TA_FUSED", "1") != "0"
_TA_FUSED_C = tuple(int(k) for k in os.environ.get("DC_TA_FUSED_C", "320,640").split(","))
_FFP_FUSED = os.environ.get("DC_FFP_FUSED", "1") != "0"
_TC_FUSED = os.environ.get("DC_TC_FUSED", "1") != "0"
_FUSED_MIN_ROWS = int(os.environ.get("DC_FUSED_MIN_ROWS", "4096"))
_LN_FUSED_K = tuple(int(k) for k in os.environ.get("DC_LN_FUSED_K", "320,640").split(","))
C_IN_PAD = 64


def _block_layout(cfg):
# ... 177 lines not shown
        self.temporal_attention, self.temporal_length = temporal_attention, temporal_length
        self.addition_attention = addition_attention
        self.image_cross_attention = image_cross_attention
        self.image_cross_attention_scale_learnable = image_cross_attention_scale_learnable
        self.default_fs, self.fs_condition = default_fs, fs_condition
        self.context_dim = context_dim
        self.dtype = torch.float32
        self._cfg = dict(in_channels=in_channels, out_channels=out_channels, model_channels=model_channels,
                         attention_resolutions=list(attention_resolutions), num_res_blocks=num_res_blocks,
                         channel_mult=list(channel_mult), num_head_channels=num_head_channels,
                         context_dim=context_dim, temporal_conv=temporal_conv, temporal_attention=temporal_attention,
                         addition_attention=addition_attention, image_cross_attention=image_cross_attention,
                         image_cross_attention_scale_learnable=image_cross_attention_scale_learnable,
                         fs_condition=fs_condition, use_linear=use_linear)
        self._layout = _block_layout(self._cfg)
        self._cat_plan = self._make_cat_plan()
        attach_params(self, _shape_table(self._cfg))
        self._packed = None
        self._arena = _Arena()
        self.register_load_state_dict_post_hook(lambda m, k: setattr(m, "_packed", None))

    def _make_cat_plan(self):
        down_path, middle, up_path = self._layout
        out_ch = lambda blk: [a.get("cout", a.get("ch")) for k, a in blk if k in ("conv_in", "res", "down", "up")][-1]
        widths = [out_ch(b) for b in down_path]
        ch = out_ch(middle)
        plan = []
        for blk in up_path:
            skip = widths.pop()
            assert blk[0][1]["cin"] == ch + skip
            plan.append((ch, skip))
            ch = out_ch(blk)
        return plan

    def _p(self, name):
        node = self
        parts = name.split(".")
        for s in parts[:-1]:
            node = node._modules[s]
        return node._parameters[parts[-1]]

    def _has(self, name):
        node = self
        parts = name.split(".")
        for s in parts[:-1]:
            node = node._modules.get(s)
            if node is None:
                return False
        return parts[-1] in node._parameters

    def invalidate_packed(self):
        self._packed = None

    def _pack(self, device):
        P = {}
        f32 = lambda n: self._p(n).detach().to(device=device, dtype=torch.float32).contiguous()
        lin = lambda n: PackedWeight.linear(self._p(n + ".weight"), self._p(n + ".bias") if self._has(n + ".bias") else None, device)

        def attn_self(p):
            w = torch.cat([self._p(f"{p}.to_{x}.weight") for x in "qkv"], dim=0)
            return {"qkv": PackedWeight.linear(w, None, device), "out": lin(p + ".to_out.0")}

        def tblock(p, cross):
            d = {"attn1": attn_self(p + ".attn1"), "ff1": lin(p + ".ff.net.0.proj"), "ff2": lin(p + ".ff.net.2")}
            if d["ff2"].N == 320 and d["ff1"].N == 2560:
                d["ff2p"] = ops.ff2_permuted(self._p(p + ".ff.net.2.weight"), device)
            for n in ("norm1", "norm2", "norm3"):
                d[n] = (f32(f"{p}.{n}.weight"), f32(f"{p}.{n}.bias"))
            if cross:
                a = p + ".attn2"
                d["q2"] = lin(a + ".to_q")
                names = ["to_k", "to_v"] + (["to_k_ip", "to_v_ip"] if self.image_cross_attention else [])
                d["kv_ctx"] = PackedWeight.linear(torch.cat([self._p(f"{a}.{x}.weight") for x in names], 0), None, device)
                d["out2"] = lin(a + ".to_out.0")
                d["ip_scale"] = 1.0
                if self.image_cross_attention and self.image_cross_attention_scale_learnable:
                    d["ip_scale"] = float(torch.tanh(self._p(a + ".alpha").detach().float()).item() + 1.0)
            else:
                d["attn2"] = attn_self(p + ".attn2")
            d["key"] = p
            return d

        def with_projp(d, p):
            w = self._p(p + ".proj_out.weight")
            if "ff2p" in d["blk"] and w.shape[0] == 320 and w[0].numel() == 320:
                d["proj_p"] = ops.ff2_permuted(w.reshape(320, 320), device)
            return d

        def temporal(p):
            return with_projp({"norm": (f32(p + ".norm.weight"), f32(p + ".norm.bias")), "proj_in": lin(p + ".proj_in"),
                               "blk": tblock(p + ".transformer_blocks.0", False), "proj_out": lin(p + ".proj_out")}, p)

        P["time0"], P["time2"] = lin("time_embed.0"), lin("time_embed.2")
        if self.fs_condition:
            P["fps0"], P["fps2"] = lin("fps_embedding.0"), lin("fps_embedding.2")
        if self.addition_attention:
            P["init_attn"] = temporal("init_attn.0")

        def pack_block(prefix, blk):
            out = []
            for j, (kind, a) in enumerate(blk):
                p = f"{prefix}.{j}"
                if kind == "conv_in":
                    d = {"conv": PackedWeight.conv3x3(self._p(p + ".weight"), self._p(p + ".bias"), device)}
                    if a["cin"] <= 8 and os.environ.get("DC_CONVIN_IM2COL", "1") != "0":
                        d["lin8"] = PackedWeight.conv3x3_c8_as_linear(self._p(p + ".weight"), self._p(p + ".bias"), device)
                    out.append(d)
                elif kind == "res":
                    d = {"gn1": (f32(p + ".in_layers.0.weight"), f32(p + ".in_layers.0.bias")),
                         "conv1": PackedWeight.conv3x3(self._p(p + ".in_layers.2.weight"), self._p(p + ".in_layers.2.bias"), device),
                         "emb": lin(p + ".emb_layers.1"),
                         "gn2": (f32(p + ".out_layers.0.weight"), f32(p + ".out_layers.0.bias")),
                         "conv2": PackedWeight.conv3x3(self._p(p + ".out_layers.3.weight"), self._p(p + ".out_layers.3.bias"), device)}
                    if a["cin"] != a["cout"]:
                        d["skip"] = lin(p + ".skip_connection")
                    if a["tconv"]:
                        d["tc"] = []
                        for i, ci in ((1, 2), (2, 3), (3, 3), (4, 3)):
                            q = f"{p}.temopral_conv.conv{i}"
                            d["tc"].append(((f32(q + ".0.weight"), f32(q + ".0.bias")),
                                            PackedWeight.tconv3(self._p(f"{q}.{ci}.weight"), self._p(f"{q}.{ci}.bias"), device)))
                    out.append(d)
                elif kind == "spatial":
                    out.append(with_projp({"norm": (f32(p + ".norm.weight"), f32(p + ".norm.bias")), "proj_in": lin(p + ".proj_in"),
                                           "blk": tblock(p + ".transformer_blocks.0", True), "proj_out": lin(p + ".proj_out")}, p))
                elif kind == "temporal":
                    out.append(temporal(p))
                elif kind == "down":
                    out.append({"conv": PackedWeight.conv3x3(self._p(p + ".op.weight"), self._p(p + ".op.bias"), device)})
                elif kind == "up":
                    out.append({"conv": PackedWeight.conv3x3(self._p(p + ".conv.weight"), self._p(p + ".conv.bias"), device)})
            return out

        down_path, middle, up_path = self._layout
        P["in"] = [pack_block(f"input_blocks.{i}", b) for i, b in enumerate(down_path)]
        P["mid"] = pack_block("middle_block", middle)
        P["out"] = [pack_block(f"output_blocks.{i}", b) for i, b in enumerate(up_path)]
        P["out_gn"] = (f32("out.0.weight"), f32("out.0.bias"))
        P["out_conv"] = PackedWeight.conv3x3(self._p("out.2.weight"), self._p("out.2.bias"), device, n_align=4)
        P["device"] = device
        self._pack_gen = getattr(self, "_pack_gen", 0) + 1
        P["gen"] = self._pack_gen
        return P

    def packed(self, device):
        if self._packed is None or self._packed["device"] != device:
            self._packed = self._pack(device)
        return self._packed

    def _gn(self, x, wb, tag, *, n_inst, rpi, eps, silu):
        y = self._arena.get(tag, x.shape[0], x.shape[1], device=x.device)
        return ops.groupnorm(x, y, wb[0], wb[1], groups=32, n_inst=n_inst, rows_per_inst=rpi, eps=eps, silu=silu)

    def _ln(self, x, wb, tag):
        y = self._arena.get(tag, x.shape[0], x.shape[1], device=x.device)
        return ops.layernorm(x, y, wb[0], wb[1], 1e-5)

    def _res(self, W, x, g, out_tag, out=None):
        A = self._arena
        M, dev = x.shape[0], x.device
        cout = W["conv1"].N
        conv = dict(IH=g["H"], IW=g["W"], OH=g["H"], OW=g["W"], stride=1, pad=1, ups=0)
        emb_out = A.get("emb_out", g["B"], cout, torch.float32, dev)
        ops.gemv_small(g["emb"], W["emb"], emb_out, act_in=1)
        h = self._gn(x, W["gn1"], "gn", n_inst=g["F"], rpi=g["HW"], eps=1e-5, silu=True)
        h1 = ops.gemm(h, W["conv1"], A.get("res_h1", M, cout, device=dev), conv=conv, rowvec=emb_out,
                      rows_per_vec=g["T"] * g["HW"])
        h = self._gn(h1, W["gn2"], "gn", n_inst=g["F"], rpi=g["HW"], eps=1e-5, silu=True)
        skip = x
        if "skip" in W:
            skip = ops.gemm(x, W["skip"], A.get("res_skip", M, cout, device=dev))
        has_tc = "tc" in W
        final = (lambda: out if out is not None else A.get(out_tag, M, cout, device=dev))
        h2 = ops.gemm(h, W["conv2"], A.get("res_h2", M, cout, device=dev) if has_tc else final(), conv=conv,
                      residual=skip)
        if not has_tc:
            return h2
        tc = dict(T=g["T"], HW=g["HW"])
        r = h2
        fused_tc = (_TC_FUSED and cout in _LN_FUSED_K and g["T"] == 16 and g["HW"] % 8 == 0 and M >= _FUSED_MIN_ROWS
                    and (g["T"] * g["HW"]) % 128 == 0)
        for i, (gnw, cw) in enumerate(W["tc"]):
            last = i == 3
            dst = final() if last else A.get("res_ta" if i % 2 == 0 else "res_tb", M, cout, device=dev)
            if fused_tc:
                st = A.get("gn_stats", g["B"] * 32 * 2, 1, torch.float32, dev)
                ops.groupnorm_stats(r, st, groups=32, n_inst=g["B"], rows_per_inst=g["T"] * g["HW"], eps=1e-5)
                r = ops.gn_silu_tconv3(r, gnw[0], gnw[1], st, cw, dst, B=g["B"], T=16, HW=g["HW"],
                                           residual=h2 if last else None)
                continue
            n = self._gn(r, gnw, "gn", n_inst=g["B"], rpi=g["T"] * g["HW"], eps=1e-5, silu=True)
            r = ops.gemm(n, cw, dst, tconv=tc, residual=h2 if last else None)
        return r

    def _ln_linear(self, h, ln, pw, out):
        if _LN_FUSED and pw.K in _LN_FUSED_K and pw.N % 32 == 0 and h.shape[0] >= _FUSED_MIN_ROWS:
            return ops.ln_linear(h, pw, out, ln=ln, ln_eps=1e-5)
        return ops.gemm(self._ln(h, ln, "ln"), pw, out)

    def _lin_res(self, x, pw, res, out):
        if _LR_FUSED and pw.K in _LN_FUSED_K and pw.N % 32 == 0 and x.shape[0] >= _FUSED_MIN_ROWS:
            return ops.linear_residual(x, pw, res, out)
        return ops.gemm(x, pw, out, residual=res)

    def _gn_linear(self, x, gnw, pw, out, *, n_inst, rpi):
        if _LN_FUSED and pw.K in _LN_FUSED_K and pw.N % 32 == 0 and x.shape[0] >= _FUSED_MIN_ROWS and rpi % 128 == 0:
            st = self._arena.get("gn_stats", n_inst * 32 * 2, 1, torch.float32, x.device)
            ops.groupnorm_stats(x, st, groups=32, n_inst=n_inst, rows_per_inst=rpi, eps=1e-6)
            return ops.gn_linear(x, gnw[0], gnw[1], st, pw, out, groups=32, rows_per_inst=rpi)
        return ops.gemm(self._gn(x, gnw, "gn", n_inst=n_inst, rpi=rpi, eps=1e-6, silu=False), pw, out)

    def _attn_self_spatial(self, Wa, ln, h, g, heads):
        A = self._arena
        M, dev, Cc = h.shape[0], h.device, heads * 64
        qkv = self._ln_linear(h, ln, Wa["qkv"], A.get("qkv", M, 3 * Cc, device=dev))
        att = A.get("att", M, Cc, device=dev)
        ops.flash_attn(qkv[:, :Cc], qkv[:, Cc:2 * Cc], qkv[:, 2 * Cc:], att, batch=g["F"], heads=heads, Lq=g["HW"],
                       Lk=g["HW"], scale=0.125)
        return self._lin_res(att, Wa["out"], h, h)

    def _attn_self_temporal(self, Wa, ln, h, g, heads):
        A = self._arena
        M, dev, Cc = h.shape[0], h.device, heads * 64
        att = A.get("att", M, Cc, device=dev)
        if _TA_FUSED and Cc in _TA_FUSED_C and g["T"] == 16 and g["HW"] % 8 == 0 and M >= _FUSED_MIN_ROWS:
            ops.ln_qkv_temporal_attn(h, ln, Wa["qkv"], att, B=g["B"], T=16, HW=g["HW"], scale=0.125)
            return self._lin_res(att, Wa["out"], h, h)
        qkv = self._ln_linear(h, ln, Wa["qkv"], A.get("qkv", M, 3 * Cc, device=dev))
        ops.temporal_attn(qkv, att, B=g["B"], T=g["T"], HW=g["HW"], heads=heads, scale=0.125)
        return self._lin_res(att, Wa["out"], h, h)

    def _ff(self, Wb, h, tag="ln"):
        A = self._arena
        if "ff2p" in Wb and _FF_FUSED and h.shape[0] >= _FUSED_MIN_ROWS:
            return ops.ff_geglu_fused320(h, Wb["ff1"], Wb["ff2p"], Wb["ff2"].bias, h, residual=h, ln=Wb["norm3"], ln_eps=1e-5)
        n = self._ln(h, Wb["norm3"], tag)
        mid = ops.gemm(n, Wb["ff1"], A.get("ffmid", h.shape[0], Wb["ff1"].N // 2, device=h.device), geglu=True)
        return ops.gemm(mid, Wb["ff2"], h, residual=h)

    def _ff_proj(self, W, h, x, out):
        B_ = W["blk"]
        if "proj_p" in W and _FF_FUSED and _FFP_FUSED and h.shape[0] >= _FUSED_MIN_ROWS:
            return ops.ff_geglu_proj_fused320(h, B_["ff1"], B_["ff2p"], B_["ff2"].bias, W["proj_p"], W["proj_out"].bias, x, out,
                                              ln=B_["norm3"], ln_eps=1e-5)
        h = self._ff(B_, h)
        return self._lin_res(h, W["proj_out"], x, out)

    def _spatial_pre(self, W, x, g, heads):
        A = self._arena
        M, dev, Cc = x.shape[0], x.device, x.shape[1]
        h = self._gn_linear(x, W["norm"], W["proj_in"], A.get("tr_h", M, Cc, device=dev), n_inst=g["F"], rpi=g["HW"])
        B_ = W["blk"]
        return self._attn_self_spatial(B_["attn1"], B_["norm1"], h, g, heads)

    def _context_kv(self, B_, ctx, tag):
        return ops.gemm(ctx, B_["kv_ctx"], self._arena.get(tag, ctx.shape[0], B_["kv_ctx"].N, device=ctx.device))

    def precompute_context_kv(self, ctx_rows):
        Wt = self.packed(ctx_rows.device)
        down_path, middle, up_path = self._layout
        out = {"__gen__": Wt["gen"]}
        for name, blks, Ws in (("in", down_path, Wt["in"]), ("mid", [middle], [Wt["mid"]]), ("out", up_path, Wt["out"])):
            for i, (blk, Wb) in enumerate(zip(blks, Ws)):
                for j, ((kind, a), W) in enumerate(zip(blk, Wb)):
                    if kind == "spatial":
                        out[W["blk"]["key"]] = self._context_kv(W["blk"], ctx_rows, f"kvctx.{name}{i}.{j}")
        return out

    def _spatial_post(self, W, x, h, g, heads, out_tag, out=None):
        A = self._arena
        M, dev, Cc = x.shape[0], x.device, x.shape[1]
        B_ = W["blk"]
        q = self._ln_linear(h, B_["norm2"], B_["q2"], A.get("q2", M, Cc, device=dev))
        kv = None if g.get("ctx_kv") is None else g["ctx_kv"].get(B_["key"])
        if kv is None:
            kv = self._context_kv(B_, g["ctx"], "kvctx")
        att = A.get("att", M, Cc, device=dev)
        Lc, nt = g["Lc"], g["n_text"]
        if self.image_cross_attention and Lc > nt:
            ops.cross_attn_dual(q, kv[:, :Cc], kv[:, Cc:2 * Cc], kv[nt:, 2 * Cc:3 * Cc], kv[nt:, 3 * Cc:], att, batch=g["F"],
                                heads=heads, Lq=g["HW"], Lk=nt, Lk2=Lc - nt, scale=0.125, scale2=B_["ip_scale"], kv_bstride=Lc)
        else:
            ops.flash_attn(q, kv[:, :Cc], kv[:, Cc:2 * Cc], att, batch=g["F"], heads=heads, Lq=g["HW"], Lk=nt, scale=0.125,
                           kv_bstride=Lc)
        h = self._lin_res(att, B_["out2"], h, h)
        return self._ff_proj(W, h, x, out if out is not None else A.get(out_tag, M, Cc, device=dev))

    def _spatial(self, W, x, g, heads, out_tag, out=None):
        return self._spatial_post(W, x, self._spatial_pre(W, x, g, heads), g, heads, out_tag, out=out)

    def _temporal(self, W, x, g, heads, out_tag, out=None):
        A = self._arena
        M, dev, Cc = x.shape[0], x.device, x.shape[1]
        inner = W["proj_in"].N
        h = self._gn_linear(x, W["norm"], W["proj_in"], A.get("tr_h", M, inner, device=dev), n_inst=g["B"],
                            rpi=g["T"] * g["HW"])
        B_ = W["blk"]
        h = self._attn_self_temporal(B_["attn1"], B_["norm1"], h, g, heads)
        h = self._attn_self_temporal(B_["attn2"], B_["norm2"], h, g, heads)
        return self._ff_proj(W, h, x, out if out is not None else A.get(out_tag, M, Cc, device=dev))

    def _run_block(self, blk, Wb, h, g, tag, final=None):
        A = self._arena
        for j, ((kind, a), W) in enumerate(zip(blk, Wb)):
            out_tag = f"{tag}.{j}"
            dev = h.device
            last = final is not None and j == len(blk) - 1
            if kind == "conv_in":
                conv = dict(IH=g["H"], IW=g["W"], OH=g["H"], OW=g["W"], stride=1, pad=1, ups=0)
                dst = final(h.shape[0], a["cout"]) if last else A.get(out_tag, h.shape[0], a["cout"], device=dev)
                if "lin8" in W:
                    cols = ops.im2col3x3_c8(h, A.get(out_tag + ".im2col", h.shape[0], 128, device=dev), n_img=h.shape[0] // (g["H"] * g["W"]),
                                            H=g["H"], W=g["W"])
                    h = ops.gemm(cols, W["lin8"], dst)
                else:
                    h = ops.gemm(h, W["conv"], dst, conv=conv)
            elif kind == "res":
                h = self._res(W, h, g, out_tag, out=final(h.shape[0], a["cout"]) if last else None)
            elif kind == "spatial":
                h = self._spatial(W, h, g, a["heads"], out_tag, out=final(h.shape[0], a["ch"]) if last else None)
            elif kind == "temporal":
                h = self._temporal(W, h, g, a["heads"], out_tag, out=final(h.shape[0], a["ch"]) if last else None)
            elif kind == "down":
                OH, OW = (g["H"] + 1) // 2, (g["W"] + 1) // 2
                conv = dict(IH=g["H"], IW=g["W"], OH=OH, OW=OW, stride=2, pad=1, ups=0)
                rows = g["F"] * OH * OW
                h = ops.gemm(h, W["conv"], final(rows, a["ch"]) if last else A.get(out_tag, rows, a["ch"], device=dev), conv=conv)
                g["H"], g["W"], g["HW"] = OH, OW, OH * OW
            elif kind == "up":
                OH, OW = g["H"] * 2, g["W"] * 2
                conv = dict(IH=g["H"], IW=g["W"], OH=OH, OW=OW, stride=1, pad=1, ups=1)
                rows = g["F"] * OH * OW
                h = ops.gemm(h, W["conv"], final(rows, a["ch"]) if last else A.get(out_tag, rows, a["ch"], device=dev), conv=conv)
                g["H"], g["W"], g["HW"] = OH, OW, OH * OW
        return h

    def _replicate(self, src, tag, nrep, dst=None):
        if dst is None:
            dst = self._arena.get(tag, nrep * src.shape[0], src.shape[1], device=src.device)
        for k in range(nrep):
            ops.copy2d(src, dst[k * src.shape[0]:(k + 1) * src.shape[0]])
        return dst

    def forward_rows(self, xrows, t_table, ctx_rows, *, B, T, H, W, Lc, n_text=77, fs_table=None, t_index=None,
                     shared_prefix=1, ctx_kv=None):
# ... 140 lines not shown
```

### dynamicrafter_amd/ops.py

```python
import ctypes as C
import os
import math

import torch

from . import _hip
from ._hip import DcDdimParams, DcGemmParams, check

_BF16 = torch.bfloat16


def stream_ptr():
    return C.c_void_p(torch.cuda.current_stream().cuda_stream)


class Tracer:

    def __init__(self):
        self.records = []

    def __enter__(self):
        global _TRACE
        _TRACE = self
        return self

    def __exit__(self, *a):
        global _TRACE
        _TRACE = None

    def _event(self):
        e = C.c_void_p()
        check(_hip.lib().dc_event_create(C.byref(e)), "dc_event_create")
        return e

    def summary(self):
        l = _hip.lib()
        out = {}
        self.detail = {}
        for name, flops, nbytes, e0, e1, tag in self.records:
            ms = C.c_float()
            check(l.dc_event_elapsed_ms(e0, e1, C.byref(ms)), "dc_event_elapsed_ms")
            d = out.setdefault(name, dict(launches=0, ms=0.0, flops=0.0, bytes=0.0))
            d["launches"] += 1; d["ms"] += ms.value; d["flops"] += flops; d["bytes"] += nbytes
            if tag is not None:
                dd = self.detail.setdefault((name, tag), dict(launches=0, ms=0.0, flops=0.0))
                dd["launches"] += 1; dd["ms"] += ms.value; dd["flops"] += flops
            l.dc_event_destroy(e0); l.dc_event_destroy(e1)
        self.records = []
        return out


_TRACE = None


def _launch(name, flops, nbytes, fn, *args, tag=None):
    tr = _TRACE
    if tr is None:
        check(fn(*args), name)
        return
    l = _hip.lib()
    e0, e1 = tr._event(), tr._event()
    sp = stream_ptr()
    l.dc_event_record(e0, sp)
    check(fn(*args), name)
    l.dc_event_record(e1, sp)
    if name == "dc_gemm_conv":
        name = l.dc_gemm_last_variant().decode()
    tr.records.append((name, flops, nbytes, e0, e1, tag))


def _ptr(t):
    return C.c_void_p(0 if t is None else t.data_ptr())


def _rows(t, name="tensor", dtype=_BF16):
    if t.dtype != dtype or t.dim() != 2 or t.stride(1) != 1 or not t.is_cuda:
        raise ValueError(f"{name}: expected CUDA {dtype} rows [R, C] with unit column stride, got "
                         f"{t.dtype} {tuple(t.shape)} strides {t.stride()} on {t.device}")
    return t


class PackedWeight:

    __slots__ = ("w", "bias", "N", "K", "n_pad", "Cin", "taps", "k_real")

    def __init__(self, w, bias, N, K, Cin, taps, k_real=None):
        self.w, self.bias, self.N, self.K, self.Cin, self.taps = w, bias, N, K, Cin, taps
        self.n_pad = w.shape[0]
        self.k_real = k_real

    @staticmethod
    def _finish(w2d, bias, device, Cin, taps, pad_n_to=None):
        N, K = w2d.shape
        n_pad = (N + 127) // 128 * 128
        if pad_n_to is not None:
            n_pad = max(n_pad, pad_n_to)
        wp = torch.zeros((n_pad, K), dtype=_BF16, device=device)
        wp[:N] = w2d.to(device=device, dtype=_BF16)
        b = None if bias is None else bias.detach().to(device=device, dtype=torch.float32).contiguous()
        return PackedWeight(wp, b, N, K, Cin, taps)

    @staticmethod
    def linear(weight, bias, device, n_align=1):
        w = weight.detach().reshape(weight.shape[0], -1)
        N, K = w.shape
        if K % 64 != 0:
            kp = (K + 63) // 64 * 64
            w = torch.nn.functional.pad(w, (0, kp - K))
        if N % n_align != 0:
            npad = (N + n_align - 1) // n_align * n_align
            w = torch.nn.functional.pad(w, (0, 0, 0, npad - N))
            if bias is not None:
                bias = torch.nn.functional.pad(bias.detach(), (0, npad - N))
        return PackedWeight._finish(w, bias, device, w.shape[1], 1)

    @staticmethod
    def conv3x3(weight, bias, device, n_align=1):
        co, ci = weight.shape[0], weight.shape[1]
        w = weight.detach().permute(0, 2, 3, 1)
        cip = (ci + 63) // 64 * 64
        if cip != ci:
            w = torch.nn.functional.pad(w, (0, cip - ci))
        w = w.reshape(co, 9, cip // 64, 64).permute(0, 2, 1, 3).reshape(co, 9 * cip)
        if co % n_align != 0:
            npad = (co + n_align - 1) // n_align * n_align
            w = torch.nn.functional.pad(w, (0, 0, 0, npad - co))
            if bias is not None:
                bias = torch.nn.functional.pad(bias.detach(), (0, npad - co))
        pw = PackedWeight._finish(w, bias, device, cip, 9)
        pw.k_real = 9 * ci
        return pw

    @staticmethod
    def conv3x3_c8_as_linear(weight, bias, device):
        co, ci = weight.shape[0], weight.shape[1]
        assert ci <= 8
        w = torch.zeros(co, 16, 8, dtype=weight.dtype)
        w[:, :9, :ci] = weight.detach().permute(0, 2, 3, 1).reshape(co, 9, ci)
        pw = PackedWeight._finish(w.reshape(co, 128), bias, device, 128, 1)
        pw.k_real = 9 * ci
        return pw

    @staticmethod
    def tconv3(weight, bias, device):
        co, ci = weight.shape[0], weight.shape[1]
        assert ci % 64 == 0, "temporal conv width must be a multiple of 64"
        w = weight.detach().reshape(co, ci // 64, 64, 3).permute(0, 1, 3, 2).reshape(co, 3 * ci)
        return PackedWeight._finish(w, bias, device, ci, 3)


def gemm(a, pw, out, *, M=None, residual=None, rowvec=None, rows_per_vec=1, geglu=False, gelu=False, alpha=1.0,
         conv=None, tconv=None):
    _rows(a, "a")
    out_f32 = out.dtype == torch.float32
    if not out_f32:
        _rows(out, "out")
    p = DcGemmParams()
    p.A, p.W, p.C = a.data_ptr(), pw.w.data_ptr(), out.data_ptr()
    p.bias = 0 if pw.bias is None else pw.bias.data_ptr()
    p.rowvec = 0 if rowvec is None else rowvec.data_ptr()
    p.rowvec_ld = 0 if rowvec is None else rowvec.stride(0)
    p.rows_per_vec = rows_per_vec
    p.residual = 0 if residual is None else _rows(residual, "residual").data_ptr()
    p.ldr = 0 if residual is None else residual.stride(0)
    p.lda, p.ldc = a.stride(0), out.stride(0)
    p.M = out.shape[0] if M is None else M
    p.N, p.K, p.n_pad = pw.N, pw.K, pw.n_pad
    p.Cin = pw.Cin
    p.flags = (_hip.DC_GEMM_OUT_F32 if out_f32 else 0) | (_hip.DC_GEMM_GEGLU if geglu else 0) | \
        (_hip.DC_GEMM_GELU if gelu else 0)
    p.alpha = alpha
    ws = _gemm_workspace(a.device, torch.cuda.current_stream().cuda_stream)
    p.workspace, p.workspace_bytes = ws.data_ptr(), ws.numel()
    if conv is not None:
        p.mode = 1
        p.IH, p.IW, p.OH, p.OW = conv["IH"], conv["IW"], conv["OH"], conv["OW"]
        p.stride, p.pad, p.ups = conv.get("stride", 1), conv.get("pad", 1), conv.get("ups", 0)
        if pw.taps != 9 or a.shape[1] < pw.Cin:
            raise ValueError("conv3x3 weight / activation mismatch")
    elif tconv is not None:
        p.mode = 2
        p.T, p.HW = tconv["T"], tconv["HW"]
        if pw.taps != 3:
            raise ValueError("tconv weight mismatch")
    else:
        p.mode = 0
        if a.shape[1] < pw.K:
            raise ValueError(f"gemm: activation has {a.shape[1]} columns, weight K={pw.K}")
    n_out = pw.N // 2 if geglu else pw.N
    if out.shape[1] < n_out:
        raise ValueError(f"gemm: out has {out.shape[1]} columns, need {n_out}")
    if out.shape[0] < p.M or (residual is not None and (residual.shape[0] < p.M or residual.shape[1] < n_out)):
        raise ValueError(f"gemm: out/residual have fewer than M={p.M} rows (or residual fewer than {n_out} columns)")
    if p.mode == 1:
        if p.M % (p.OH * p.OW) != 0 or a.shape[0] < (p.M // (p.OH * p.OW)) * p.IH * p.IW:
            raise ValueError(f"conv3x3: M={p.M} output rows need {p.M // (p.OH * p.OW)} frames of {p.IH}x{p.IW} input rows, "
                             f"activation has {a.shape[0]}")
    elif a.shape[0] < p.M:
        raise ValueError(f"gemm: activation has {a.shape[0]} rows, M={p.M}")
    if p.mode == 2 and (p.M % (p.T * p.HW) != 0 or a.shape[1] < pw.Cin):
        raise ValueError("tconv: M must be a multiple of T*HW and the activation at least Cin wide")
    if rowvec is not None and (rowvec.shape[0] * rows_per_vec < p.M or rowvec.shape[1] < n_out):
        raise ValueError("gemm: rowvec does not cover every row group / output column")
    if _TRACE is not None:
        variant = "dc_gemm_conv"
        k_real = pw.k_real if pw.k_real else pw.K
        flops = 2.0 * p.M * pw.N * k_real
        esz = 4 if out_f32 else 2
        nbytes = 2.0 * p.M * (k_real if p.mode == 0 else pw.Cin) + 2.0 * pw.N * pw.K + esz * p.M * n_out \
            + (2.0 * p.M * n_out if residual is not None else 0)
        _launch(variant, flops, nbytes, _hip.lib().dc_gemm_conv, C.byref(p), stream_ptr(),
                tag=(p.mode, p.M, pw.N, k_real))
    else:
        check(_hip.lib().dc_gemm_conv(C.byref(p), stream_ptr()), "dc_gemm_conv")
    return out


_gemm_ws = {}


def _gemm_workspace(device, stream):
    key = (device.index, stream)
    buf = _gemm_ws.get(key)
    if buf is None:
        buf = torch.empty(int(_hip.lib().dc_gemm_workspace_bytes()), dtype=torch.uint8, device=device)
        _gemm_ws[key] = buf
    return buf


class Arena:
    GUARD = 8

    def __init__(self):
        self._bufs = {}
        self._guarded = {}
        self.guard = os.environ.get("DC_ARENA_GUARD", "0") == "1"

    def get(self, tag, rows, cols, dtype=_BF16, device=None, zero=False):
        key = (tag, rows, cols, dtype)
        b = self._bufs.get(key)
        if b is None:
            if rows * cols >= 2 ** 31:
                raise ValueError(f"scratch buffer {tag} [{rows} x {cols}] has 2^31 elements or more")
            if self.guard:
                G = self.GUARD
                whole = torch.empty((rows + 2 * G, cols), dtype=dtype, device=device)
                whole.fill_(self._sentinel(dtype))
                b = whole[G:G + rows]
                if zero:
                    b.zero_()
                self._guarded[key] = whole
            else:
                b = (torch.zeros if zero else torch.empty)((rows, cols), dtype=dtype, device=device)
            self._bufs[key] = b
        return b

    @staticmethod
    def _sentinel(dtype):
        return 12345.0 if dtype.is_floating_point else 0x5a

    def check(self):
        bad = []
        for (tag, rows, cols, dtype), whole in self._guarded.items():
            G = self.GUARD
            ref = torch.full((1,), self._sentinel(dtype), dtype=dtype, device=whole.device)
            if not (bool((whole[:G] == ref).all()) and bool((whole[G + rows:] == ref).all())):
                bad.append(f"{tag}[{rows}x{cols} {dtype}]")
        if bad:
            raise RuntimeError("scratch buffers overrun: " + ", ".join(bad))
        return len(self._guarded)

    def nbytes(self):
        return sum(b.numel() * b.element_size() for b in self._bufs.values())


_gn_ws = {}


_gn_ws_retired = []


def _gn_workspace(device, nbytes):
    key = (device.index, torch.cuda.current_stream().cuda_stream)
    buf = _gn_ws.get(key)
    if buf is None or buf.numel() * 4 < nbytes:
        if buf is not None:
            _gn_ws_retired.append(buf)
        buf = torch.empty((max(nbytes, 4 << 20) + 3) // 4, dtype=torch.float32, device=device)
        _gn_ws[key] = buf
    return buf


def _need(t, n, name):
    if t is not None and t.numel() < n:
        raise ValueError(f"{name}: {t.numel()} elements, the launch reads/writes {n}")


def _need_rows(t, rows, cols, name):
    if t.shape[0] < rows or t.shape[1] < cols:
        raise ValueError(f"{name}: shape {tuple(t.shape)}, the launch addresses [{rows}, {cols}]")


def groupnorm(x, y, gamma, beta, *, groups, n_inst, rows_per_inst, eps, silu):
    _rows(x, "x"); _rows(y, "y")
    _need_rows(x, n_inst * rows_per_inst, gamma.numel(), "x"); _need_rows(y, n_inst * rows_per_inst, gamma.numel(), "y")
    _need(beta, gamma.numel(), "beta")
    Cc = gamma.numel()
    l = _hip.lib()
    ws = _gn_workspace(x.device, int(l.dc_groupnorm_workspace_bytes(n_inst, groups, rows_per_inst)))
    _launch("groupnorm(2-3 kernels)", 0.0, 6.0 * n_inst * rows_per_inst * Cc, l.dc_groupnorm, _ptr(x), x.stride(0), _ptr(y),
            y.stride(0), _ptr(gamma), _ptr(beta), Cc, groups, n_inst, rows_per_inst, eps, 1 if silu else 0, _ptr(ws),
            stream_ptr())
    return y


def layernorm(x, y, gamma, beta, eps=1e-5):
    _rows(x, "x"); _rows(y, "y")
    _need_rows(x, x.shape[0], gamma.numel(), "x"); _need_rows(y, x.shape[0], gamma.numel(), "y"); _need(beta, gamma.numel(), "beta")
    _launch("layernorm", 0.0, 4.0 * x.shape[0] * gamma.numel(), _hip.lib().dc_layernorm, _ptr(x), x.stride(0), _ptr(y),
            y.stride(0), _ptr(gamma), _ptr(beta), x.shape[0], gamma.numel(), eps, stream_ptr())
    return y


def flash_attn(q, k, v, o, *, batch, heads, Lq, Lk, scale, accumulate=False, acc_scale=1.0, q_bstride=None,
               kv_bstride=None):
    for t, n in ((q, "q"), (k, "k"), (v, "v"), (o, "o")):
        _rows(t, n)
    qb = Lq if q_bstride is None else q_bstride
    kb = Lk if kv_bstride is None else kv_bstride
    _need_rows(q, (batch - 1) * qb + Lq, heads * 64, "q"); _need_rows(o, (batch - 1) * qb + Lq, heads * 64, "o")
    _need_rows(k, (batch - 1) * kb + Lk, heads * 64, "k"); _need_rows(v, (batch - 1) * kb + Lk, heads * 64, "v")
    _launch("flash_attn_d64(self)" if Lk > 128 else "flash_attn_d64(cross)", 4.0 * batch * heads * Lq * Lk * 64,
            2.0 * batch * heads * 64 * (2 * Lq + 2 * Lk), _hip.lib().dc_flash_attn_d64, _ptr(q), _ptr(k), _ptr(v), _ptr(o),
            q.stride(0), k.stride(0), v.stride(0), o.stride(0), batch, heads, Lq, Lk,
            Lq if q_bstride is None else q_bstride, Lk if kv_bstride is None else kv_bstride, scale,
            1 if accumulate else 0, acc_scale, stream_ptr())
    return o


def cross_attn_dual(q, k, v, k2, v2, o, *, batch, heads, Lq, Lk, Lk2, scale, scale2, kv_bstride):
    for t, n in ((q, "q"), (k, "k"), (v, "v"), (k2, "k2"), (v2, "v2"), (o, "o")):
        _rows(t, n)
    if len({k.stride(0), v.stride(0), k2.stride(0), v2.stride(0)}) != 1:
        raise ValueError("cross_attn_dual: k, v, k2, v2 must share one row stride")
    _need_rows(q, batch * Lq, heads * 64, "q"); _need_rows(o, batch * Lq, heads * 64, "o")
    _need_rows(k, (batch - 1) * kv_bstride + Lk, heads * 64, "k"); _need_rows(v, (batch - 1) * kv_bstride + Lk, heads * 64, "v")
    _need_rows(k2, (batch - 1) * kv_bstride + Lk2, heads * 64, "k2"); _need_rows(v2, (batch - 1) * kv_bstride + Lk2, heads * 64, "v2")
    _launch("flash_attn_d64(cross)", 4.0 * batch * heads * Lq * (Lk + Lk2) * 64, 2.0 * batch * heads * 64 * (2 * Lq + 2 * (Lk + Lk2)),
            _hip.lib().dc_cross_attn_dual_d64, _ptr(q), _ptr(k), _ptr(v), _ptr(k2), _ptr(v2), _ptr(o), q.stride(0), k.stride(0),
            o.stride(0), batch, heads, Lq, Lk, Lk2, Lq, kv_bstride, scale, scale2, stream_ptr())
    return o


def temporal_attn(qkv, o, *, B, T, HW, heads, scale):
    _rows(qkv, "qkv"); _rows(o, "o")
    _need_rows(qkv, B * T * HW, 3 * heads * 64, "qkv"); _need_rows(o, B * T * HW, heads * 64, "o")
    _launch("temporal_attn_d64", 4.0 * B * HW * heads * T * T * 64, 2.0 * B * T * HW * heads * 64 * 4,
            _hip.lib().dc_temporal_attn_d64, _ptr(qkv), qkv.stride(0), _ptr(o), o.stride(0), B, T, HW, heads, scale,
            stream_ptr())
    return o


def ff2_permuted(weight, device):
    w = weight.detach()
    N, K = w.shape
    pos = torch.arange(32)
    s_, h_, e_ = pos // 16, (pos // 8) % 2, pos % 8
    chan = 8 * (2 * s_ + e_ // 4) + 4 * h_ + e_ % 4
    idx = (torch.arange(K // 32)[:, None] * 32 + chan[None, :]).reshape(-1)
    n_pad = (N + 127) // 128 * 128
    out = torch.zeros((n_pad, K), dtype=_BF16, device=device)
    out[:N] = w[:, idx].to(device=device, dtype=_BF16)
    return out


def ff_geglu_fused320(x, pw1, w2p, b2, out, residual=None, ln=None, ln_eps=1e-5):
    _rows(x, "x"); _rows(out, "out")
    M = x.shape[0]
    if pw1.K != 320 or pw1.N != 2560 or pw1.bias is None or tuple(w2p.shape[1:]) != (1280,) or w2p.shape[0] < 320:
        raise ValueError("ff_geglu_fused320: dim must be 320 (ff1 [2560, 320] with bias, ff2 [320, 1280])")
    _need_rows(x, M, 320, "x"); _need_rows(out, M, 320, "out")
    if residual is not None:
        _rows(residual, "residual"); _need_rows(residual, M, 320, "residual")
    if ln is not None:
        _need(ln[0], 320, "ln gamma"); _need(ln[1], 320, "ln beta")
    flops = 2.0 * M * (2560 + 1280) * 320
    nbytes = 2.0 * M * 320 * (3 if residual is not None else 2) + 2.0 * (2560 * 320 + 320 * 1280)
    _launch("ff_geglu_fused320", flops, nbytes, _hip.lib().dc_ff_geglu_fused320, _ptr(x), x.stride(0),
            _ptr(None if ln is None else ln[0]), _ptr(None if ln is None else ln[1]), ln_eps, _ptr(pw1.w), _ptr(pw1.bias),
            _ptr(w2p), _ptr(b2), _ptr(residual), 0 if residual is None else residual.stride(0), _ptr(out), out.stride(0), M,
            stream_ptr())
    return out


def ff_geglu_proj_fused320(x, pw1, w2p, b2, wp, bp, residual2, out, ln=None, ln_eps=1e-5):
    _rows(x, "x"); _rows(out, "out"); _rows(residual2, "residual2")
    M = x.shape[0]
    if pw1.K != 320 or pw1.N != 2560 or pw1.bias is None or tuple(w2p.shape[1:]) != (1280,) or w2p.shape[0] < 320 \
            or tuple(wp.shape[1:]) != (320,) or wp.shape[0] < 320:
        raise ValueError("ff_geglu_proj_fused320: dim must be 320 (ff1 [2560, 320] with bias, ff2 [320, 1280], proj [320, 320])")
    if x.data_ptr() == out.data_ptr():
        raise ValueError("ff_geglu_proj_fused320: out must not alias x")
    _need_rows(x, M, 320, "x"); _need_rows(out, M, 320, "out"); _need_rows(residual2, M, 320, "residual2")
    _need(b2, 320, "b2"); _need(bp, 320, "bp")
    if ln is not None:
        _need(ln[0], 320, "ln gamma"); _need(ln[1], 320, "ln beta")
    _launch("ff_geglu_proj_fused320", 2.0 * M * (2560 + 1280 + 320) * 320, 2.0 * M * 320 * 3 + 2.0 * (2560 * 320 + 320 * 1280 + 320 * 320),
            _hip.lib().dc_ff_geglu_proj_fused320, _ptr(x), x.stride(0), _ptr(None if ln is None else ln[0]),
            _ptr(None if ln is None else ln[1]), ln_eps, _ptr(pw1.w), _ptr(pw1.bias), _ptr(w2p), _ptr(b2), _ptr(wp), _ptr(bp),
            _ptr(residual2), residual2.stride(0), _ptr(out), out.stride(0), M, stream_ptr())
    return out


def ln_linear(x, pw, out, ln=None, ln_eps=1e-5):
    _rows(x, "x"); _rows(out, "out")
    M, K = x.shape[0], pw.K
    if K not in (320, 640) or pw.N % 32:
        raise ValueError("ln_linear: K must be 320 or 640 and N a multiple of 32")
    _need_rows(x, M, K, "x"); _need_rows(out, M, pw.N, "out")
    if ln is not None:
        _need(ln[0], K, "ln gamma"); _need(ln[1], K, "ln beta")
    _launch("ln_linear", 2.0 * M * pw.N * K, 2.0 * M * (K + pw.N) + 2.0 * pw.N * K, _hip.lib().dc_ln_linear,
            _ptr(x), x.stride(0), K, _ptr(None if ln is None else ln[0]), _ptr(None if ln is None else ln[1]), ln_eps,
            _ptr(pw.w), _ptr(pw.bias), _ptr(out), out.stride(0), M, pw.N, stream_ptr())
    return out


def linear_residual(x, pw, residual, out):
    _rows(x, "x"); _rows(out, "out"); _rows(residual, "residual")
    M, K = x.shape[0], pw.K
    if K not in (320, 640) or pw.N % 32:
        raise ValueError("linear_residual: K must be 320 or 640 and N a multiple of 32")
    _need_rows(x, M, K, "x"); _need_rows(out, M, pw.N, "out"); _need_rows(residual, M, pw.N, "residual")
    _launch("linear_residual", 2.0 * M * pw.N * K, 2.0 * M * (K + 2 * pw.N) + 2.0 * pw.N * K, _hip.lib().dc_linear_residual,
            _ptr(x), x.stride(0), K, _ptr(pw.w), _ptr(pw.bias), _ptr(residual), residual.stride(0), _ptr(out), out.stride(0),
            M, pw.N, stream_ptr())
    return out


def ln_qkv_temporal_attn(x, ln, pw_qkv, out, *, B, T, HW, scale, ln_eps=1e-5):
    _rows(x, "x"); _rows(out, "out")
    M = B * T * HW
    Cc = pw_qkv.K
    if Cc not in (320, 640) or pw_qkv.N != 3 * Cc or pw_qkv.bias is not None or T != 16 or HW % 8:
        raise ValueError("ln_qkv_temporal_attn: dim 320 / 640 (qkv weight [3 C, C], no bias), T = 16, HW % 8 == 0")
    if x.data_ptr() == out.data_ptr():
        raise ValueError("ln_qkv_temporal_attn: out must not alias x")
    _need_rows(x, M, Cc, "x"); _need_rows(out, M, Cc, "out"); _need(ln[0], Cc, "ln gamma"); _need(ln[1], Cc, "ln beta")
    fn = _hip.lib().dc_ln_qkv_temporal_attn320 if Cc == 320 else _hip.lib().dc_ln_qkv_temporal_attn640
    _launch(f"ln_qkv_temporal_attn{Cc}", 2.0 * M * 3 * Cc * Cc + 4.0 * M * T * Cc, 4.0 * M * Cc + 2.0 * 3 * Cc * Cc,
            fn, _ptr(x), x.stride(0), _ptr(ln[0]), _ptr(ln[1]), ln_eps, _ptr(pw_qkv.w),
            _ptr(out), out.stride(0), B, T, HW, scale, stream_ptr())
    return out


def gn_silu_tconv3(x, gamma, beta, stats, pw, out, *, B, T, HW, groups=32, residual=None):
    _rows(x, "x"); _rows(out, "out")
    M = B * T * HW
    C = pw.w.shape[1] // 3
    if C not in (320, 640) or pw.w.shape[1] != 3 * C or pw.N % 32 or pw.bias is None or T != 16 or HW % 8:
        raise ValueError("gn_silu_tconv3: 320 / 640 input channels (weight [N, 3 C] with bias), N % 32 == 0, T = 16, HW % 8 == 0")
    if x.data_ptr() == out.data_ptr():
        raise ValueError("gn_silu_tconv3: out must not alias x")
    _need_rows(x, M, C, "x"); _need_rows(out, M, pw.N, "out")
    _need(gamma, C, "gamma"); _need(beta, C, "beta"); _need(stats, B * groups * 2, "stats")
# ... 557 lines not shown
```

### include/dcrafter_hip.h

```cpp
#ifndef DCRAFTER_HIP_H
#define DCRAFTER_HIP_H
#include <stdint.h>

#ifdef __cplusplus
extern "C" {
#endif

#define DC_ERR_SHAPE (-1)
#define DC_ERR_ARG   (-2)

#define DC_GEMM_OUT_F32 1
#define DC_GEMM_GEGLU   2
#define DC_GEMM_GELU    4

typedef struct DcGemmParams {
    const uint16_t* A;
    const uint16_t* W;
    void* C;
    const float* bias;
    const float* rowvec;
    const uint16_t* residual;
    int lda, ldc, ldr, rowvec_ld;
    int rows_per_vec;
    int M, N, K, n_pad;
    int mode;
    int Cin;
    int IH, IW, OH, OW;
    int stride, pad, ups;
    int T, HW;
    int flags;
    float alpha;
    void* workspace;
    long long workspace_bytes;
} DcGemmParams;

const char* dc_gemm_last_variant(void);

int dc_gemm_set_plan(int plan);

int64_t dc_gemm_workspace_bytes(void);

int dc_gemm_conv(const DcGemmParams* p, void* stream);

int dc_groupnorm(const uint16_t* x, int ldx, uint16_t* y, int ldy, const float* gamma, const float* beta,
                 int C, int groups, int n_inst, int rows_per_inst, float eps, int silu,
                 float* workspace, void* stream);
int64_t dc_groupnorm_workspace_bytes(int n_inst, int groups, int rows_per_inst);

int dc_layernorm(const uint16_t* x, int ldx, uint16_t* y, int ldy, const float* gamma, const float* beta,
                 int rows, int C, float eps, void* stream);

int dc_flash_attn_d64(const uint16_t* q, const uint16_t* k, const uint16_t* v, uint16_t* o,
                      int ldq, int ldk, int ldv, int ldo, int batch, int heads, int Lq, int Lk,
                      int64_t q_bstride, int64_t kv_bstride, float scale, int accumulate, float acc_scale,
                      void* stream);

int dc_flash_attn_set_mode(int mode, float thr);

int dc_temporal_attn_d64(const uint16_t* qkv, int ld, uint16_t* o, int ldo, int B, int T, int HW, int heads,
                         float scale, void* stream);

int dc_gemv_small(const float* in, int ld_in, const uint16_t* W, const float* bias, float* out, int ld_out,
                  int M, int N, int K, int act_in, int act_out, int accumulate, void* stream);

int dc_timestep_embedding(const int64_t* t_table, const int32_t* t_index, int t_stride, float* out, int B, int dim,
                          float max_period, void* stream);

int dc_pack_latent(const float* x, const float* cc, uint16_t* out, int B, int Cx, int Cc, int T, int HW,
                   int c_pad, int nrep, void* stream);

int dc_pack_latent_windows(const float* x, const float* cc, uint16_t* out, const int32_t* starts,
                           const int32_t* step_index, int index, int S, int W, int w0, int n_w, int B, int Cx, int Cc,
                           int T_long, int T, int HW, int c_pad, int nrep, void* stream);

int dc_window_merge(const float* e, int ld_e, float* out, int ld_out, const int32_t* starts, const float* wn,
                    const int32_t* step_index, int index, int S, int W, int w0, int n_w, int nb, int B, int C, int T_long,
                    int T, int HW, int accumulate, void* stream);

int dc_nchw_to_rows(const float* x, uint16_t* out, int N, int C, int HW, int c_pad, float scale, void* stream);
int dc_rows_to_nchw(const void* rows, int ld, int rows_f32, float* y, int N, int C, int HW, float scale, void* stream);

int dc_im2col3x3_c8(const uint16_t* x, int ldx, uint16_t* out, int ldo, int n_img, int H, int W, void* stream);

int dc_copy2d(const uint16_t* src, int lds, uint16_t* dst, int ldd, int rows, int cols, void* stream);

int dc_build_context(const float* ctx, uint16_t* out, int B, int T, int n_text, int L, int D, void* stream);

int dc_softmax_rows(const float* x, int ldx, uint16_t* y, int ldy, int rows, int cols, void* stream);

int dc_transpose(const uint16_t* src, int lds, uint16_t* dst, int ldd, int rows, int cols, void* stream);

int dc_add_rows(const uint16_t* a, int lda, const uint16_t* b, int ldb, uint16_t* y, int ldy, int rows, int cols,
                void* stream);

int dc_vae_sample(const uint16_t* moments, int ld, const float* noise, float* z, int N, int zc, int HW,
                  float scale, void* stream);

typedef struct DcDdimParams {
    const float* a_t;
    const float* a_prev;
    const float* sigma_t;
    const float* sqrt_one_minus_at;
    const float* sqrt_acp_t;
    const float* sqrt_1macp_t;
    const float* scale_ratio;
    const int32_t* step_index;
    int index;
    int v_param;
    float cfg_scale;
    float cfg_img;
    float guidance_rescale;
    float temperature;
    int e_nchw;
    int64_t noise_step_stride;
} DcDdimParams;

int dc_ddim_step(const DcDdimParams* p, const float* e_cond, const float* e_uncond, const float* e_img, int ld_e,
                 const float* x, const float* noise, float* x_prev, float* pred_x0, int B, int C, int THW,
                 float* workspace, void* stream);

typedef struct DcDpmParams {
    const float* A;
    const float* alpha_t;
    const float* alpha_p_r;
    const float* k;
    const float* N;
    const float* sqrt_one_minus_at;
    const float* sqrt_acp_t;
    const float* sqrt_1macp_t;
    const float* scale_ratio;
    const int32_t* step_index;
    int index;
    int v_param;
    float cfg_scale;
    float cfg_img;
    float guidance_rescale;
    float temperature;
    int e_nchw;
    int64_t noise_step_stride;
    float* x0_hist;
} DcDpmParams;

int dc_dpmpp_step(const DcDpmParams* p, const float* e_cond, const float* e_uncond, const float* e_img, int ld_e,
                  const float* x, const float* noise, float* x_prev, float* pred_x0, int B, int C, int THW,
                  float* workspace, void* stream);

typedef struct DcSdsParams {
    const float* c1;
    const float* c2;
    const float* w;
    const float* step_size;
    const float* bc2_sqrt;
    const int32_t* step_index;
    int index;
    int weight_type;
    int x0_param;
    int e_nchw;
    float cfg_scale;
    float guidance_rescale;
    float beta2, eps;
    float one_minus_beta1;
    float one_minus_beta2;
    float decay;
    float grad_scale;
    int64_t noise_step_stride;
    float* loss;
} DcSdsParams;

int dc_sds_noise(const DcSdsParams* p, const float* latent, const float* noise, float* x_t, int B, int64_t n_per_clip,
                 void* stream);

int dc_sds_step(const DcSdsParams* p, const float* e_cond, const float* e_uncond, int ld_e, const float* x_t,
                float* latent, float* m, float* v, int B, int C, int THW, float* workspace, void* stream);

int dc_cross_attn_dual_d64(const uint16_t* q, const uint16_t* k, const uint16_t* v, const uint16_t* k2, const uint16_t* v2,
                           uint16_t* o, int ldq, int ldkv, int ldo, int batch, int heads, int Lq, int Lk, int Lk2,
                           int64_t q_bstride, int64_t kv_bstride, float scale, float scale2, void* stream);

int dc_ff_geglu_fused320(const uint16_t* x, int ldx, const float* ln_gamma, const float* ln_beta, float ln_eps,
                         const uint16_t* w1, const float* b1, const uint16_t* w2p, const float* b2, const uint16_t* residual,
                         int ldr, uint16_t* out, int ldo, int M, void* stream);

int dc_ff_geglu_proj_fused320(const uint16_t* x, int ldx, const float* ln_gamma, const float* ln_beta, float ln_eps,
                              const uint16_t* w1, const float* b1, const uint16_t* w2p, const float* b2, const uint16_t* wp,
                              const float* bp, const uint16_t* residual2, int ldr2, uint16_t* out, int ldo, int M, void* stream);

int dc_ln_linear(const uint16_t* x, int ldx, int K, const float* ln_gamma, const float* ln_beta, float ln_eps, const uint16_t* w,
                 const float* bias, uint16_t* out, int ldo, int M, int N, void* stream);
int dc_groupnorm_stats(const uint16_t* x, int ldx, int C, int groups, int n_inst, int rows_per_inst, float eps,
                       float* workspace, float* stats_out, void* stream);
int dc_gn_linear(const uint16_t* x, int ldx, int K, const float* gamma, const float* beta, const float* stats, int groups,
                 int rows_per_inst, const uint16_t* w, const float* bias, uint16_t* out, int ldo, int M, int N, void* stream);

int dc_linear_residual(const uint16_t* x, int ldx, int K, const uint16_t* w, const float* bias, const uint16_t* residual, int ldr,
                       uint16_t* out, int ldo, int M, int N, void* stream);

int dc_ln_qkv_temporal_attn320(const uint16_t* x, int ldx, const float* ln_gamma, const float* ln_beta, float ln_eps,
                               const uint16_t* wqkv, uint16_t* out, int ldo, int B, int T, int HW, float scale, void* stream);
// ... 68 lines not shown
```

Before: 2.653 frames/s.

## Have groupnorm write a tiled activation layout consumed directly by conv GEMMs

Adds a tiled A layout (16-row by 32-channel blocks) that GroupNorm+SiLU can emit and the pipe320x16 conv/temporal-conv GEMM kernel can read directly. Halo offsets for the 3x3 taps are precomputed per row. A heuristic decides per shape when the tiled path is used. The aim is more contiguous, LDS-friendly A loads in the conv GEMMs, at the cost of extra code paths and layout coupling between the producer and consumer kernels.

```diff
diff --git a/dynamicrafter_amd/_hip.py b/dynamicrafter_amd/_hip.py
--- a/dynamicrafter_amd/_hip.py
+++ b/dynamicrafter_amd/_hip.py
@@ -8,6 +8,7 @@
 DC_GEMM_OUT_F32 = 1
 DC_GEMM_GEGLU = 2
 DC_GEMM_GELU = 4
+DC_GEMM_A_TILED = 8
 
 
 class DcGemmParams(C.Structure):
@@ -63,10 +64,14 @@
 _P, _I, _F, _L = C.c_void_p, C.c_int, C.c_float, C.c_int64
 SIGNATURES = {
     "dc_gemm_conv": (_I, [C.POINTER(DcGemmParams), _P]),
+    "dc_gemm_accepts_tiled_a": (_I, [C.POINTER(DcGemmParams)]),
+    "dc_act_tiled_set": (_I, [_I]),
+    "dc_act_tiled_offset": (_L, [_L, _I, _I]),
+    "dc_gemm_pipe16_direct": (_I, [C.POINTER(DcGemmParams), _I, _I, _I, _P]),
     "dc_gemm_workspace_bytes": (_L, []),
     "dc_gemm_last_variant": (C.c_char_p, []),
     "dc_gemm_set_plan": (_I, [_I]),
-    "dc_groupnorm": (_I, [_P, _I, _P, _I, _P, _P, _I, _I, _I, _I, _F, _I, _P, _P]),
+    "dc_groupnorm": (_I, [_P, _I, _P, _I, _P, _P, _I, _I, _I, _I, _F, _I, _I, _P, _P]),
     "dc_groupnorm_workspace_bytes": (_L, [_I, _I, _I]),
     "dc_layernorm": (_I, [_P, _I, _P, _I, _P, _P, _I, _I, _F, _P]),
     "dc_flash_attn_d64": (_I, [_P, _P, _P, _P, _I, _I, _I, _I, _I, _I, _I, _I, _L, _L, _F, _I, _F, _P]),
diff --git a/dynamicrafter_amd/csrc/dc_common.h b/dynamicrafter_amd/csrc/dc_common.h
--- a/dynamicrafter_amd/csrc/dc_common.h
+++ b/dynamicrafter_amd/csrc/dc_common.h
@@ -95,6 +95,10 @@
     return base + idx;
 }
 
+__host__ __device__ inline size_t dc_tiled_offset(size_t row, int ch, int C) {
+    return ((row >> 4) * (size_t)(C >> 5) + (size_t)(ch >> 5)) * 1024 + (size_t)((((ch & 31) >> 3) << 4) + (int)(row & 15)) * 16 + (size_t)(ch & 7) * 2;
+}
+
 void dc_note_variant(const char* name);
 
 int dc_gemm_plan_now();
diff --git a/dynamicrafter_amd/csrc/gemm_conv.hip b/dynamicrafter_amd/csrc/gemm_conv.hip
--- a/dynamicrafter_amd/csrc/gemm_conv.hip
+++ b/dynamicrafter_amd/csrc/gemm_conv.hip
@@ -549,6 +549,7 @@
 }
 
 int dc_gemm_conv_glds_try(const DcGemmParams& p, hipStream_t stream);
+bool dc_gemm_tiled_a_ok(const DcGemmParams& p);
 
 static bool glds_enabled() {
     static int v = -1;
@@ -567,18 +568,50 @@
     return (int64_t)8 * 40 * 256 * 320 * 4;
 }
 
+static bool shape_valid(const DcGemmParams& p) {
+    if (p.M <= 0 || p.N <= 0 || p.K <= 0) return false;
+    if (p.K % BK != 0 || p.N % 4 != 0 || p.lda % 8 != 0 || p.ldc % 4 != 0) return false;
+    if (p.mode != 0 && (p.Cin % BK != 0)) return false;
+    if (p.mode == 1 && p.K != 9 * p.Cin) return false;
+    if (p.mode == 2 && p.K != 3 * p.Cin) return false;
+    if (p.residual && (p.ldr % 4 != 0)) return false;
+    const bool geglu = (p.flags & DC_GEMM_GEGLU) != 0;
+    if (geglu && ((p.N / 2) % 64 != 0 || p.n_pad < p.N)) return false;
+    if (p.n_pad < (p.N + 127) / 128 * 128) return false;
+    return true;
+}
+
+static bool tiled_a_route(const DcGemmParams& p) {
+    return shape_valid(p) && !narrow_conv_ok(p) && !window128_conv_ok(p) && glds_enabled() && dc_gemm_tiled_a_ok(p);
+}
+
+extern "C" int64_t dc_act_tiled_offset(int64_t row, int ch, int C) {
+    if (row < 0 || ch < 0 || ch >= C || C % 64 != 0) return -1;
+    return (int64_t)dc_tiled_offset((size_t)row, ch, C);
+}
+
+static bool tiled_a_pays(const DcGemmParams& p) {
+    return p.mode == 2 || (p.mode == 1 && p.Cin >= 640 && p.Cin <= 1920 && p.M >= 16384);
+}
+
+static std::atomic<int> g_act_tiled{[] { const char* e = getenv("DC_ACT_TILED"); return (e && e[0] >= '0' && e[0] <= '2') ? e[0] - '0' : 1; }()};
+
+extern "C" int dc_act_tiled_set(int mode) {
+    if (mode < 0 || mode > 2) return DC_ERR_ARG;
+    return g_act_tiled.exchange(mode, std::memory_order_relaxed);
+}
+
+extern "C" int dc_gemm_accepts_tiled_a(const DcGemmParams* pp) {
+    const int mode = g_act_tiled.load(std::memory_order_relaxed);
+    return (pp && mode && tiled_a_route(*pp) && (mode == 2 || tiled_a_pays(*pp))) ? 1 : 0;
+}
+
 extern "C" int dc_gemm_conv(const DcGemmParams* pp, void* stream_) {
     const DcGemmParams& p = *pp;
     hipStream_t stream = (hipStream_t)stream_;
-    if (p.M <= 0 || p.N <= 0 || p.K <= 0) return DC_ERR_SHAPE;
-    if (p.K % BK != 0 || p.N % 4 != 0 || p.lda % 8 != 0 || p.ldc % 4 != 0) return DC_ERR_SHAPE;
-    if (p.mode != 0 && (p.Cin % BK != 0)) return DC_ERR_SHAPE;
-    if (p.mode == 1 && p.K != 9 * p.Cin) return DC_ERR_SHAPE;
-    if (p.mode == 2 && p.K != 3 * p.Cin) return DC_ERR_SHAPE;
-    if (p.residual && (p.ldr % 4 != 0)) return DC_ERR_SHAPE;
+    if (!shape_valid(p)) return DC_ERR_SHAPE;
+    if ((p.flags & DC_GEMM_A_TILED) && !tiled_a_route(p)) return DC_ERR_SHAPE;
     const bool geglu = (p.flags & DC_GEMM_GEGLU) != 0;
-    if (geglu && ((p.N / 2) % 64 != 0 || p.n_pad < p.N)) return DC_ERR_SHAPE;
-    if (p.n_pad < (p.N + 127) / 128 * 128) return DC_ERR_SHAPE;
     if (narrow_conv_ok(p)) return launch_narrow_conv(p, stream);
     if (window128_conv_ok(p)) return launch_window128_conv(p, stream);
     if (glds_enabled()) {
diff --git a/dynamicrafter_amd/csrc/gemm_conv_glds.hip b/dynamicrafter_amd/csrc/gemm_conv_glds.hip
--- a/dynamicrafter_amd/csrc/gemm_conv_glds.hip
+++ b/dynamicrafter_amd/csrc/gemm_conv_glds.hip
@@ -827,12 +827,13 @@
 int launch_pipe_shape(const DcGemmParams& p, hipStream_t stream, GemmSplit sp, int gx, int gy) {
     sp.err = dc_error_word_device();
     if (!sp.err) return DC_ERR_ARG;
+    if constexpr (MODE == 1 || MODE == 2)
+        if (p.flags & DC_GEMM_A_TILED) return launch_pipe320x16<MODE, EPI, true>(p, stream, sp, gx, gy);
     return launch_pipe320x16<MODE, EPI>(p, stream, sp, gx, gy);
 }
 
-inline bool pipe_ok(const DcGemmParams& p, int plan) {
-    if (!(plan & 3) || (!(plan & 2) && p.mode != 1)) return false;
-    if (p.mode != 1 && p.K < pipe_min_k()) return false;
+inline bool pipe_addressable(const DcGemmParams& p) {
+    if (p.M <= 0 || p.K <= 0) return false;
     if (p.flags & (DC_GEMM_GEGLU | DC_GEMM_OUT_F32)) return false;
     if (p.ups && !(p.mode == 1 && p.ups == 1 && p.stride == 1 && p.pad == 1 && p.OH == 2 * p.IH && p.OW == 2 * p.IW)) return false;
     if (p.N % 320 != 0 || p.n_pad < p.N || p.K % 64 != 0 || p.lda % 8 != 0 || ((uintptr_t)p.A % 16) != 0) return false;
@@ -845,6 +846,12 @@
     if ((rows + extra) * p.lda * 2 >= (1ll << 31)) return false;
     if (320ll * p.K * 2 >= (1ll << 31)) return false;
     return true;
+}
+
+inline bool pipe_ok(const DcGemmParams& p, int plan) {
+    if (!(plan & 3) || (!(plan & 2) && p.mode != 1)) return false;
+    if (p.mode != 1 && p.K < pipe_min_k()) return false;
+    return pipe_addressable(p);
 }
 
 int launch_pipe_whole(const DcGemmParams& p, hipStream_t stream) {
@@ -923,13 +930,69 @@
 
 inline float wave_eff(int wgs) { return (float)wgs / (float)(((wgs + 255) / 256) * 256); }
 
+struct Choice320 { int w320, w128, full, splits; float waste128, s320, s128; };
+inline int splitk_on() { static const int v = [] { const char* e = getenv("DC_GEMM_SPLITK"); return e ? atoi(e) : 1; }(); return v; }
+
+inline Choice320 choose320(const DcGemmParams& p, bool use_pipe, int force) {
+    Choice320 c;
+    const int tiles_m = (p.M + GBM - 1) / GBM;
+    const int t128 = (p.N + 127) / 128;
+    const bool n320 = (p.N % 320 == 0) && (p.n_pad >= p.N);
+    const int w320 = n320 ? tiles_m * (p.N / 320) : 0;
+    const int w128 = tiles_m * t128;
+    const float waste128 = (float)(t128 * 128) / (float)p.N;
+    const bool pipe_conv = use_pipe && p.mode == 1 && force == 0;
+    float s320 = n320 ? (pipe_conv ? 1.4f : 1.25f) * wave_eff(w320) : 0.f;
+    float s128 = wave_eff(w128) / waste128;
+    if (w320 < (pipe_conv ? 128 : 200)) s320 = 0.f;
+    if (w128 < 384) s128 = 0.f;
+    c.w320 = w320; c.w128 = w128; c.waste128 = waste128; c.s320 = s320; c.s128 = s128; c.full = 0; c.splits = 0;
+    if (splitk_on() && force == 0 && n320 && p.workspace && p.n_pad >= p.N) {
+        const int nk = p.K / GBK;
+        int full = 0, splits = 0;
+        if (w320 < 200 && w320 >= 8) {
+            splits = 256 / w320;
+            if (splits > 12) splits = 12;
+            while (splits > 2 && nk / splits < 12) --splits;
+        } else if (w320 > 256 && w320 <= 1280 && (w320 % 256) != 0 && (w320 % 256) <= 128) {
+            full = (w320 / 256) * 256;
+            splits = 256 / (w320 - full);
+            if (splits > 8) splits = 8;
+            while (splits > 2 && nk / splits < 8) --splits;
+        }
+        const size_t need = (size_t)splits * (size_t)(w320 - full) * GBM * 320 * sizeof(float);
+        if (splits >= 2 && nk / splits >= (full ? 8 : 12) && need <= (size_t)p.workspace_bytes) { c.full = full; c.splits = splits; }
+    }
+    return c;
+}
+
+inline int force_tile() { static const int v = [] { const char* e = getenv("DC_GEMM_TILE"); return e ? atoi(e) : 0; }(); return v; }
+
+inline bool tiled_a_shape(const DcGemmParams& p) {
+    if (p.lda != p.Cin || p.M % 16 != 0) return false;
+    if (p.mode == 1) return !p.ups && p.stride == 1 && p.pad == 1 && p.OH == p.IH && p.OW == p.IW && p.IW % 16 == 0;
+    if (p.mode == 2) return p.HW % 16 == 0;
+    return false;
+}
+
+}
+
+bool dc_gemm_tiled_a_ok(const DcGemmParams& p) {
+    if (!tiled_a_shape(p) || force_tile() != 0) return false;
+    if (!pipe_ok(p, g_gemm_plan.load(std::memory_order_relaxed))) return false;
+    const Choice320 ch = choose320(p, true, 0);
+    return ch.splits >= 2 || (ch.s320 > 0.f && ch.s320 >= ch.s128);
+}
+
+namespace {
+
 }
 
 int dc_gemm_conv_glds_try(const DcGemmParams& p, hipStream_t stream) {
     const bool geglu = (p.flags & DC_GEMM_GEGLU) != 0;
     const int n_out = geglu ? p.N / 2 : p.N;
     const int tiles_m = (p.M + GBM - 1) / GBM;
-    static const int force = [] { const char* e = getenv("DC_GEMM_TILE"); return e ? atoi(e) : 0; }();
+    static const int force = force_tile();
     static const int persist = [] { const char* e = getenv("DC_GEMM_PERSIST"); return e ? atoi(e) : 1; }();
     if (geglu && p.mode != 0) return DC_ERR_ARG;
     const bool out_f32 = (p.flags & DC_GEMM_OUT_F32) != 0;
@@ -968,39 +1031,18 @@
         if (w128 < 384) return -100;
         return launch_glds<128, true, 0, 3>(p, stream);
     }
-    const int t128 = (p.N + 127) / 128;
-    const bool n320 = (p.N % 320 == 0) && (p.n_pad >= p.N);
-    const int w320 = n320 ? tiles_m * (p.N / 320) : 0;
-    const int w128 = tiles_m * t128;
-    const float waste128 = (float)(t128 * 128) / (float)p.N;
-    const bool pipe_conv = use_pipe && p.mode == 1 && force == 0;
-    float s320 = n320 ? (pipe_conv ? 1.4f : 1.25f) * wave_eff(w320) : 0.f;
-    float s128 = wave_eff(w128) / waste128;
-    if (w320 < (pipe_conv ? 128 : 200)) s320 = 0.f;
-    if (w128 < 384) s128 = 0.f;
-    static const int splitk = [] { const char* e = getenv("DC_GEMM_SPLITK"); return e ? atoi(e) : 1; }();
-    if (splitk && force == 0 && n320 && p.workspace && p.n_pad >= p.N) {
-        const int nk = p.K / GBK;
-        int full = 0, splits = 0;
-        if (w320 < 200 && w320 >= 8) {
-            splits = 256 / w320;
-            if (splits > 12) splits = 12;
-            while (splits > 2 && nk / splits < 12) --splits;
-        } else if (w320 > 256 && w320 <= 1280 && (w320 % 256) != 0 && (w320 % 256) <= 128) {
-            full = (w320 / 256) * 256;
-            splits = 256 / (w320 - full);
-            if (splits > 8) splits = 8;
-            while (splits > 2 && nk / splits < 8) --splits;
-        }
-        const size_t need = (size_t)splits * (size_t)(w320 - full) * GBM * 320 * sizeof(float);
-        if (splits >= 2 && nk / splits >= (full ? 8 : 12) && need <= (size_t)p.workspace_bytes) {
-            const bool merged = !(plan & 64);
-            if (p.mode == 0) return launch_glds320_split<0>(p, stream, w320, full, splits, use_pipe, merged);
-            if (p.mode == 1) return p.ups ? launch_glds320_split<3>(p, stream, w320, full, splits, use_pipe, merged)
-                                          : launch_glds320_split<1>(p, stream, w320, full, splits, use_pipe, merged);
-            return launch_glds320_split<2>(p, stream, w320, full, splits, use_pipe, merged);
-        }
-    }
+    const Choice320 ch = choose320(p, use_pipe, force);
+    const bool n320 = ch.w320 > 0;
+    const int w128 = ch.w128;
+    const float waste128 = ch.waste128, s320 = ch.s320, s128 = ch.s128;
+    if (ch.splits >= 2) {
+        const bool merged = !(plan & 64);
+        if (p.mode == 0) return launch_glds320_split<0>(p, stream, ch.w320, ch.full, ch.splits, use_pipe, merged);
+        if (p.mode == 1) return p.ups ? launch_glds320_split<3>(p, stream, ch.w320, ch.full, ch.splits, use_pipe, merged)
+                                      : launch_glds320_split<1>(p, stream, ch.w320, ch.full, ch.splits, use_pipe, merged);
+        return launch_glds320_split<2>(p, stream, ch.w320, ch.full, ch.splits, use_pipe, merged);
+    }
+    static const int splitk = splitk_on();
     static const int splitk256 = [] { const char* e = getenv("DC_GEMM_SPLITK256"); return e ? atoi(e) : 1; }();
     if (splitk && splitk256 && force == 0 && !n320 && !out_f32 && p.workspace && p.N % 256 == 0 && p.n_pad >= p.N && (p.mode != 1 || !p.ups)) {
         const int w256s = tiles_m * (p.N / 256), nk = p.K / GBK;
@@ -1027,6 +1069,22 @@
     return -100;
 }
 
+extern "C" int dc_gemm_pipe16_direct(const DcGemmParams* pp, int full, int splits, int merged, void* stream_) {
+    if (!pp) return DC_ERR_ARG;
+    const DcGemmParams& p = *pp;
+    if (!pipe_addressable(p)) return DC_ERR_SHAPE;
+    if ((p.flags & DC_GEMM_A_TILED) && !tiled_a_shape(p)) return DC_ERR_SHAPE;
+    hipStream_t stream = (hipStream_t)stream_;
+    if (splits < 2) return launch_pipe_whole(p, stream);
+    const int ntiles = ((p.M + GBM - 1) / GBM) * (p.N / 320);
+    if (full < 0 || full >= ntiles || p.K / GBK < splits || (merged && (full <= 0 || full % 8 != 0))) return DC_ERR_SHAPE;
+    if (!p.workspace || (size_t)splits * (size_t)(ntiles - full) * GBM * 320 * sizeof(float) > (size_t)p.workspace_bytes) return DC_ERR_SHAPE;
+    if (p.mode == 0) return launch_glds320_split<0>(p, stream, ntiles, full, splits, true, merged != 0);
+    if (p.mode == 1) return p.ups ? launch_glds320_split<3>(p, stream, ntiles, full, splits, true, merged != 0)
+                                  : launch_glds320_split<1>(p, stream, ntiles, full, splits, true, merged != 0);
+    return launch_glds320_split<2>(p, stream, ntiles, full, splits, true, merged != 0);
+}
+
 int dc_gemm_plan_now() { return g_gemm_plan.load(std::memory_order_relaxed); }
 
 extern "C" int dc_gemm_set_plan(int plan) {
diff --git a/dynamicrafter_amd/csrc/gemm_pipe16.h b/dynamicrafter_amd/csrc/gemm_pipe16.h
--- a/dynamicrafter_amd/csrc/gemm_pipe16.h
+++ b/dynamicrafter_amd/csrc/gemm_pipe16.h
@@ -16,7 +16,7 @@
     asm volatile("s_nop 7\n\ts_nop 7" ::: "memory");
 }
 
-template <int MODE, int EPI>
+template <int MODE, int EPI, bool TILED = false>
 __global__ __launch_bounds__(256, 1) __attribute__((amdgpu_waves_per_eu(1, 1)))
 void gemm_pipe320x16_kernel(const DcGemmParams p, const GemmSplit sp) {
     extern __shared__ __attribute__((aligned(16))) char smem[];
@@ -52,7 +52,9 @@
     unsigned rowoff[4];
     int mask[4];
     long long bias = 0;
-    if (MODE == 1) bias = (long long)(p.pad * p.IW + p.pad) * lda2;
+    if (MODE == 1) bias = TILED ? (long long)p.IW * lda2 : (long long)(p.pad * p.IW + p.pad) * lda2;
+    auto tiled_off = [&](int mm) { return (unsigned)(mm >> 4) * (lda2 * 16u) + (unsigned)(mm & 15) * 16u + lq * 256u; };
+    const int dx_m = -16 - (lr == 0 ? (int)lda2 * 16 - 256 : 0), dx_p = 16 + (lr == 15 ? (int)lda2 * 16 - 256 : 0);
     if (MODE == 2) bias = (long long)p.HW * lda2;
     if (MODE == 3) bias = (long long)(p.IW + 1) * lda2;
 #ifdef GP_DBG_QUAD_ROWS
@@ -82,7 +84,8 @@
                 if (ok && iy >= 0 && iy < p.IH && ix >= 0 && ix < p.IW) mk |= 1 << t;
             }
             mask[rb] = mk;
-            rowoff[rb] = (unsigned)(((n * p.IH + iy0 + p.pad) * p.IW + ix0 + p.pad)) * lda2 + lq_a * 16;
+            if (TILED) rowoff[rb] = tiled_off(mm);
+            else rowoff[rb] = (unsigned)(((n * p.IH + iy0 + p.pad) * p.IW + ix0 + p.pad)) * lda2 + lq_a * 16;
         } else if (MODE == 3) {
             const int ohw = p.OH * p.OW;
             const int n = mm / ohw;
@@ -106,7 +109,7 @@
                 if (ok && tt >= 0 && tt < p.T) mk |= 1 << t;
             }
             mask[rb] = mk;
-            rowoff[rb] = (unsigned)mm * lda2 + lq_a * 16;
+            rowoff[rb] = TILED ? tiled_off(mm) : (unsigned)mm * lda2 + lq_a * 16;
         }
     }
     gp_i32x4_t ars;
@@ -125,6 +128,13 @@
             const int cs = kt / 9;
             tap = kt - cs * 9;
             const int dy = tap / 3, dx = tap - dy * 3;
+            if (TILED) {
+                soff = dy * p.IW * (int)lda2 + cs * 2048;
+                const unsigned d = dx == 0 ? (unsigned)dx_m : dx == 2 ? (unsigned)dx_p : 0u;
+#pragma unroll
+                for (int rb = 0; rb < 4; ++rb) vo[rb] = ((mask[rb] >> tap) & 1) ? rowoff[rb] + d : 0x80000000u;
+                return;
+            }
             soff = (dy * p.IW + dx) * (int)lda2 + cs * 128;
         } else if (MODE == 3) {
             const int cs = kt / 9;
@@ -142,7 +152,7 @@
         } else {
             const int cs = kt / 3;
             tap = kt - cs * 3;
-            soff = tap * p.HW * (int)lda2 + cs * 128;
+            soff = tap * p.HW * (int)lda2 + cs * (TILED ? 2048 : 128);
         }
 #pragma unroll
         for (int rb = 0; rb < 4; ++rb) vo[rb] = ((mask[rb] >> tap) & 1) ? rowoff[rb] : 0x80000000u;
@@ -194,6 +204,7 @@
 #pragma unroll
         for (int i = 0; i < 8; ++i) {
             if ((i >> 2) == 0) GP_LOAD_A_(A[t][i & 3][0], vo[i & 3], ars, soff, "0");
+            else if constexpr (TILED) GP_LOAD_A_(A[t][i & 3][1], vo[i & 3], ars, soff, "1024");
             else GP_LOAD_A_(A[t][i & 3][1], vo[i & 3], ars, soff, "64");
         }
     }
@@ -256,6 +267,7 @@
                 if constexpr (g >= 90 && g <= 146 && ((g - 90) & 7) == 0) {
                     constexpr int i = (g - 90) >> 3;
                     if constexpr ((i >> 2) == 0) GP_LOAD_A_(A_[ST2][i & 3][0], vo[i & 3], ars, soff, "0");
+                    else if constexpr (TILED) GP_LOAD_A_(A_[ST2][i & 3][1], vo[i & 3], ars, soff, "1024");
                     else GP_LOAD_A_(A_[ST2][i & 3][1], vo[i & 3], ars, soff, "64");
                 }
                 if constexpr (g == 118) seen_l = *(volatile lds_int_t*)cnt_landed;
@@ -358,11 +370,11 @@
     }
 }
 
-template <int MODE, int EPI>
+template <int MODE, int EPI, bool TILED = false>
 int launch_pipe320x16(const DcGemmParams& p, hipStream_t stream, const GemmSplit& sp, int grid_x, int grid_y) {
     static DcLdsOnce lds_once;
-    if (const int e = lds_once.ensure(reinterpret_cast<const void*>(&gemm_pipe320x16_kernel<MODE, EPI>), GP_LDS)) return e;
-    hipLaunchKernelGGL((gemm_pipe320x16_kernel<MODE, EPI>), dim3(grid_x, grid_y), dim3(256), GP_LDS, stream, p, sp);
+    if (const int e = lds_once.ensure(reinterpret_cast<const void*>(&gemm_pipe320x16_kernel<MODE, EPI, TILED>), GP_LDS)) return e;
+    hipLaunchKernelGGL((gemm_pipe320x16_kernel<MODE, EPI, TILED>), dim3(grid_x, grid_y), dim3(256), GP_LDS, stream, p, sp);
     DC_CHECK_LAUNCH();
     return 0;
 }
diff --git a/dynamicrafter_amd/csrc/norms.hip b/dynamicrafter_amd/csrc/norms.hip
--- a/dynamicrafter_amd/csrc/norms.hip
+++ b/dynamicrafter_amd/csrc/norms.hip
@@ -5,6 +5,7 @@
 namespace {
 
 struct GnGeom { int chunks; int rows_per_chunk; };
+constexpr int GN_PATCH = 4 * 272;
 
 __host__ __device__ inline GnGeom gn_geom(int n_inst, int rows_per_inst) {
     int chunks = (2048 + n_inst - 1) / n_inst;
@@ -120,7 +121,7 @@
     }
 }
 
-template <bool FIN>
+template <bool FIN, bool TILED>
 __global__ void gn_apply_kernel(const bf16_t* __restrict__ x, int ldx, bf16_t* __restrict__ y, int ldy,
                                 const float* __restrict__ gamma, const float* __restrict__ beta, int C, int groups,
                                 int rows_per_inst, int rows_per_chunk, int vecs, int rpp, int silu,
@@ -170,6 +171,62 @@
         }
         __syncthreads();
     }
+    if constexpr (TILED) {
+        extern __shared__ __attribute__((aligned(16))) float scsh[];
+        const int cpg = C / groups;
+        for (int c = threadIdx.x; c < C; c += (int)blockDim.x) {
+            const float2 st = FIN ? st_s[c / cpg] : stats[(size_t)inst * groups + c / cpg];
+            const float g = gamma[c] * st.y;
+            scsh[c] = g;
+            scsh[C + c] = beta[c] - st.x * g;
+        }
+        __syncthreads();
+        const int lane = threadIdx.x & 63, unit = threadIdx.x >> 6, nunits = (int)blockDim.x >> 6;
+        const int lr = lane >> 2, lc = lane & 3;
+        char* const patch = reinterpret_cast<char*>(scsh + 2 * C) + unit * GN_PATCH;
+        const int p_wr = lc * 272 + lr * 16, p_rd = (lane >> 4) * 272 + (lane & 15) * 16;
+        const int ncb = C >> 5;
+        const int r_begin = (chunk * rows_per_chunk) & ~15;
+        int r_end = (chunk + 1) * rows_per_chunk;
+        if (r_end >= rows_per_inst) r_end = rows_per_inst; else r_end &= ~15;
+        const int ntask = ((r_end - r_begin) >> 4) * ncb;
+        const bf16_t* xb = x + ((size_t)inst * rows_per_inst + r_begin + lr) * ldx + lc * 8;
+        char* yb = reinterpret_cast<char*>(y) + (((size_t)inst * rows_per_inst + r_begin) >> 4) * ncb * 1024 + lane * 16;
+        auto src = [&](int j) -> const uint4* {
+            const int rg = j / ncb, cb = j - rg * ncb;
+            return reinterpret_cast<const uint4*>(xb + (size_t)rg * 16 * ldx + cb * 32);
+        };
+        auto apply = [&](int j, const uint4& raw) {
+            const int ch = (j % ncb) * 32 + lc * 8;
+            float f[8], sc[8], sh[8];
+            unpack_bf8(raw, f);
+            *reinterpret_cast<float4*>(sc) = *reinterpret_cast<const float4*>(scsh + ch);
+            *reinterpret_cast<float4*>(sc + 4) = *reinterpret_cast<const float4*>(scsh + ch + 4);
+            *reinterpret_cast<float4*>(sh) = *reinterpret_cast<const float4*>(scsh + C + ch);
+            *reinterpret_cast<float4*>(sh + 4) = *reinterpret_cast<const float4*>(scsh + C + ch + 4);
+#pragma unroll
+            for (int e = 0; e < 8; ++e) {
+                float t = f[e] * sc[e] + sh[e];
+                if (silu) t = silu_f(t);
+                f[e] = t;
+            }
+            *reinterpret_cast<uint4*>(patch + p_wr) = pack_bf8(f);
+            asm volatile("" ::: "memory");
+            const uint4 o = *reinterpret_cast<const uint4*>(patch + p_rd);
+            asm volatile("" ::: "memory");
+            *reinterpret_cast<uint4*>(yb + (size_t)j * 1024) = o;
+        };
+        int j = unit;
+        for (; j + 7 * nunits < ntask; j += 8 * nunits) {
+            uint4 raw[8];
+#pragma unroll
+            for (int u = 0; u < 8; ++u) raw[u] = *src(j + u * nunits);
+#pragma unroll
+            for (int u = 0; u < 8; ++u) apply(j + u * nunits, raw[u]);
+        }
+        for (; j < ntask; j += nunits) apply(j, *src(j));
+        return;
+    }
     const int v = threadIdx.x % vecs;
     const int ro = threadIdx.x / vecs;
     const int r_begin = chunk * rows_per_chunk;
@@ -285,12 +342,13 @@
 }
 
 extern "C" int dc_groupnorm(const uint16_t* x, int ldx, uint16_t* y, int ldy, const float* gamma, const float* beta,
-                            int C, int groups, int n_inst, int rows_per_inst, float eps, int silu,
+                            int C, int groups, int n_inst, int rows_per_inst, float eps, int silu, int out_tiled,
                             float* workspace, void* stream_) {
     hipStream_t stream = (hipStream_t)stream_;
     if (!x || !y || !gamma || !beta || !workspace) return DC_ERR_ARG;
     if (C % 8 != 0 || groups <= 0 || groups > 64 || C % groups != 0 || ldx % 8 != 0 || ldy % 8 != 0) return DC_ERR_SHAPE;
     if (n_inst <= 0 || rows_per_inst <= 0) return DC_ERR_SHAPE;
+    if (out_tiled && (C % 64 != 0 || C > 4096 || ldy != C || rows_per_inst % 16 != 0 || ((uintptr_t)y % 16) != 0)) return DC_ERR_SHAPE;
     const int vecs = C / 8;
     if (vecs > 1024) return DC_ERR_SHAPE;
     int rpp = 256 / vecs;
@@ -304,18 +362,27 @@
     hipLaunchKernelGGL(gn_partial_kernel, dim3(g.chunks, n_inst), dim3(threads), lds, stream, x, ldx, C, groups,
                        rows_per_inst, g.rows_per_chunk, g.chunks, vecs, rpp, partial);
     DC_CHECK_LAUNCH();
+    const size_t lds_t = (size_t)2 * C * sizeof(float) + 4 * GN_PATCH;
     static const bool fuse_fin = [] { const char* e = getenv("DC_GN_FUSE_FINALIZE"); return !(e && e[0] == '0'); }();
     if (fuse_fin && g.chunks <= 64 && threads % 8 == 0) {
-        hipLaunchKernelGGL(gn_apply_kernel<true>, dim3(g.chunks, n_inst), dim3(threads), 0, stream, x, ldx, y, ldy, gamma, beta,
-                           C, groups, rows_per_inst, g.rows_per_chunk, vecs, rpp, silu, (const float2*)partial, g.chunks, eps);
+        if (out_tiled)
+            hipLaunchKernelGGL((gn_apply_kernel<true, true>), dim3(g.chunks, n_inst), dim3(256), lds_t, stream, x, ldx, y, ldy, gamma, beta,
+                               C, groups, rows_per_inst, g.rows_per_chunk, vecs, rpp, silu, (const float2*)partial, g.chunks, eps);
+        else
+            hipLaunchKernelGGL((gn_apply_kernel<true, false>), dim3(g.chunks, n_inst), dim3(threads), 0, stream, x, ldx, y, ldy, gamma, beta,
+                               C, groups, rows_per_inst, g.rows_per_chunk, vecs, rpp, silu, (const float2*)partial, g.chunks, eps);
         DC_CHECK_LAUNCH();
         return 0;
     }
     hipLaunchKernelGGL(gn_finalize_kernel, dim3(groups, n_inst), dim3(64), 0, stream, partial, g.chunks, groups, rows_per_inst,
                        g.rows_per_chunk, C / groups, eps, stats);
     DC_CHECK_LAUNCH();
-    hipLaunchKernelGGL(gn_apply_kernel<false>, dim3(g.chunks, n_inst), dim3(threads), 0, stream, x, ldx, y, ldy, gamma, beta,
-                       C, groups, rows_per_inst, g.rows_per_chunk, vecs, rpp, silu, (const float2*)stats, g.chunks, eps);
+    if (out_tiled)
+        hipLaunchKernelGGL((gn_apply_kernel<false, true>), dim3(g.chunks, n_inst), dim3(256), lds_t, stream, x, ldx, y, ldy, gamma, beta,
+                           C, groups, rows_per_inst, g.rows_per_chunk, vecs, rpp, silu, (const float2*)stats, g.chunks, eps);
+    else
+        hipLaunchKernelGGL((gn_apply_kernel<false, false>), dim3(g.chunks, n_inst), dim3(threads), 0, stream, x, ldx, y, ldy, gamma, beta,
+                           C, groups, rows_per_inst, g.rows_per_chunk, vecs, rpp, silu, (const float2*)stats, g.chunks, eps);
     DC_CHECK_LAUNCH();
     return 0;
 }
diff --git a/dynamicrafter_amd/lvdm/modules/networks/openaimodel3d.py b/dynamicrafter_amd/lvdm/modules/networks/openaimodel3d.py
--- a/dynamicrafter_amd/lvdm/modules/networks/openaimodel3d.py
+++ b/dynamicrafter_amd/lvdm/modules/networks/openaimodel3d.py
@@ -353,6 +353,12 @@
         y = self._arena.get(tag, x.shape[0], x.shape[1], device=x.device)
         return ops.groupnorm(x, y, wb[0], wb[1], groups=32, n_inst=n_inst, rows_per_inst=rpi, eps=eps, silu=silu)
 
+    def _gn_silu_conv(self, x, wb, pw, out, *, n_inst, rpi, **kw):
+        y = self._arena.get("gn", x.shape[0], x.shape[1], device=x.device)
+        tiled = ops.gemm_accepts_tiled_a(y, pw, out, **kw)
+        ops.groupnorm(x, y, wb[0], wb[1], groups=32, n_inst=n_inst, rows_per_inst=rpi, eps=1e-5, silu=True, out_tiled=tiled)
+        return ops.gemm(y, pw, out, a_tiled=tiled, **kw)
+
     def _ln(self, x, wb, tag):
         y = self._arena.get(tag, x.shape[0], x.shape[1], device=x.device)
         return ops.layernorm(x, y, wb[0], wb[1], 1e-5)
@@ -364,17 +370,15 @@
         conv = dict(IH=g["H"], IW=g["W"], OH=g["H"], OW=g["W"], stride=1, pad=1, ups=0)
         emb_out = A.get("emb_out", g["B"], cout, torch.float32, dev)
         ops.gemv_small(g["emb"], W["emb"], emb_out, act_in=1)
-        h = self._gn(x, W["gn1"], "gn", n_inst=g["F"], rpi=g["HW"], eps=1e-5, silu=True)
-        h1 = ops.gemm(h, W["conv1"], A.get("res_h1", M, cout, device=dev), conv=conv, rowvec=emb_out,
-                      rows_per_vec=g["T"] * g["HW"])
-        h = self._gn(h1, W["gn2"], "gn", n_inst=g["F"], rpi=g["HW"], eps=1e-5, silu=True)
+        h1 = self._gn_silu_conv(x, W["gn1"], W["conv1"], A.get("res_h1", M, cout, device=dev), n_inst=g["F"], rpi=g["HW"],
+                                conv=conv, rowvec=emb_out, rows_per_vec=g["T"] * g["HW"])
         skip = x
         if "skip" in W:
             skip = ops.gemm(x, W["skip"], A.get("res_skip", M, cout, device=dev))
         has_tc = "tc" in W
         final = (lambda: out if out is not None else A.get(out_tag, M, cout, device=dev))
-        h2 = ops.gemm(h, W["conv2"], A.get("res_h2", M, cout, device=dev) if has_tc else final(), conv=conv,
-                      residual=skip)
+        h2 = self._gn_silu_conv(h1, W["gn2"], W["conv2"], A.get("res_h2", M, cout, device=dev) if has_tc else final(),
+                                n_inst=g["F"], rpi=g["HW"], conv=conv, residual=skip)
         if not has_tc:
             return h2
         tc = dict(T=g["T"], HW=g["HW"])
@@ -390,8 +394,7 @@
                 r = ops.gn_silu_tconv3(r, gnw[0], gnw[1], st, cw, dst, B=g["B"], T=16, HW=g["HW"],
                                            residual=h2 if last else None)
                 continue
-            n = self._gn(r, gnw, "gn", n_inst=g["B"], rpi=g["T"] * g["HW"], eps=1e-5, silu=True)
-            r = ops.gemm(n, cw, dst, tconv=tc, residual=h2 if last else None)
+            r = self._gn_silu_conv(r, gnw, cw, dst, n_inst=g["B"], rpi=g["T"] * g["HW"], tconv=tc, residual=h2 if last else None)
         return r
 
     def _ln_linear(self, h, ln, pw, out):
diff --git a/dynamicrafter_amd/ops.py b/dynamicrafter_amd/ops.py
--- a/dynamicrafter_amd/ops.py
+++ b/dynamicrafter_amd/ops.py
@@ -149,8 +149,37 @@
         return PackedWeight._finish(w, bias, device, ci, 3)
 
 
-def gemm(a, pw, out, *, M=None, residual=None, rowvec=None, rows_per_vec=1, geglu=False, gelu=False, alpha=1.0,
-         conv=None, tconv=None):
+def tiled_index(M, C, device=None):
+    if M % 16 != 0 or C % 64 != 0:
+        raise ValueError(f"tiled layout needs M % 16 == 0 and C % 64 == 0, got [{M}, {C}]")
+    row = torch.arange(M, device=device).unsqueeze(1)
+    ch = torch.arange(C, device=device).unsqueeze(0)
+    byte = ((row // 16) * (C // 32) + ch // 32) * 1024 + (((ch % 32) // 8) * 16 + row % 16) * 16 + (ch % 8) * 2
+    return byte // 2
+
+
+def gemm_accepts_tiled_a(a, pw, out, **kw):
+    return bool(_hip.lib().dc_gemm_accepts_tiled_a(C.byref(_gemm_params(a, pw, out, **kw)[0])))
+
+
+def gemm(a, pw, out, *, a_tiled=False, **kw):
+    p, launch = _gemm_params(a, pw, out, **kw)
+    if a_tiled:
+        p.flags |= _hip.DC_GEMM_A_TILED
+    launch(p)
+    return out
+
+
+def gemm_pipe16_direct(a, pw, out, *, full=0, splits=0, merged=True, a_tiled=False, **kw):
+    p, _ = _gemm_params(a, pw, out, **kw)
+    if a_tiled:
+        p.flags |= _hip.DC_GEMM_A_TILED
+    check(_hip.lib().dc_gemm_pipe16_direct(C.byref(p), full, splits, 1 if merged else 0, stream_ptr()), "dc_gemm_pipe16_direct")
+    return out
+
+
+def _gemm_params(a, pw, out, *, M=None, residual=None, rowvec=None, rows_per_vec=1, geglu=False, gelu=False, alpha=1.0,
+                 conv=None, tconv=None):
     _rows(a, "a")
     out_f32 = out.dtype == torch.float32
     if not out_f32:
@@ -202,18 +231,20 @@
         raise ValueError("tconv: M must be a multiple of T*HW and the activation at least Cin wide")
     if rowvec is not None and (rowvec.shape[0] * rows_per_vec < p.M or rowvec.shape[1] < n_out):
         raise ValueError("gemm: rowvec does not cover every row group / output column")
-    if _TRACE is not None:
-        variant = "dc_gemm_conv"
-        k_real = pw.k_real if pw.k_real else pw.K
-        flops = 2.0 * p.M * pw.N * k_real
-        esz = 4 if out_f32 else 2
-        nbytes = 2.0 * p.M * (k_real if p.mode == 0 else pw.Cin) + 2.0 * pw.N * pw.K + esz * p.M * n_out \
-            + (2.0 * p.M * n_out if residual is not None else 0)
-        _launch(variant, flops, nbytes, _hip.lib().dc_gemm_conv, C.byref(p), stream_ptr(),
-                tag=(p.mode, p.M, pw.N, k_real))
-    else:
-        check(_hip.lib().dc_gemm_conv(C.byref(p), stream_ptr()), "dc_gemm_conv")
-    return out
+
+    def launch(p):
+        if _TRACE is not None:
+            variant = "dc_gemm_conv"
+            k_real = pw.k_real if pw.k_real else pw.K
+            flops = 2.0 * p.M * pw.N * k_real
+            esz = 4 if out_f32 else 2
+            nbytes = 2.0 * p.M * (k_real if p.mode == 0 else pw.Cin) + 2.0 * pw.N * pw.K + esz * p.M * n_out \
+                + (2.0 * p.M * n_out if residual is not None else 0)
+            _launch(variant, flops, nbytes, _hip.lib().dc_gemm_conv, C.byref(p), stream_ptr(),
+                    tag=(p.mode, p.M, pw.N, k_real))
+        else:
+            check(_hip.lib().dc_gemm_conv(C.byref(p), stream_ptr()), "dc_gemm_conv")
+    return p, launch
 
 
 _gemm_ws = {}
@@ -301,7 +332,7 @@
         raise ValueError(f"{name}: shape {tuple(t.shape)}, the launch addresses [{rows}, {cols}]")
 
 
-def groupnorm(x, y, gamma, beta, *, groups, n_inst, rows_per_inst, eps, silu):
+def groupnorm(x, y, gamma, beta, *, groups, n_inst, rows_per_inst, eps, silu, out_tiled=False):
     _rows(x, "x"); _rows(y, "y")
     _need_rows(x, n_inst * rows_per_inst, gamma.numel(), "x"); _need_rows(y, n_inst * rows_per_inst, gamma.numel(), "y")
     _need(beta, gamma.numel(), "beta")
@@ -309,8 +340,8 @@
     l = _hip.lib()
     ws = _gn_workspace(x.device, int(l.dc_groupnorm_workspace_bytes(n_inst, groups, rows_per_inst)))
     _launch("groupnorm(2-3 kernels)", 0.0, 6.0 * n_inst * rows_per_inst * Cc, l.dc_groupnorm, _ptr(x), x.stride(0), _ptr(y),
-            y.stride(0), _ptr(gamma), _ptr(beta), Cc, groups, n_inst, rows_per_inst, eps, 1 if silu else 0, _ptr(ws),
-            stream_ptr())
+            y.stride(0), _ptr(gamma), _ptr(beta), Cc, groups, n_inst, rows_per_inst, eps, 1 if silu else 0,
+            1 if out_tiled else 0, _ptr(ws), stream_ptr())
     return y
 
 
diff --git a/include/dcrafter_hip.h b/include/dcrafter_hip.h
--- a/include/dcrafter_hip.h
+++ b/include/dcrafter_hip.h
@@ -12,6 +12,7 @@
 #define DC_GEMM_OUT_F32 1
 #define DC_GEMM_GEGLU   2
 #define DC_GEMM_GELU    4
+#define DC_GEMM_A_TILED 8
 
 typedef struct DcGemmParams {
     const uint16_t* A;
@@ -38,12 +39,18 @@
 
 int dc_gemm_set_plan(int plan);
 
+int dc_gemm_accepts_tiled_a(const DcGemmParams* p);
+int dc_act_tiled_set(int mode);
+int64_t dc_act_tiled_offset(int64_t row, int ch, int C);
+
+int dc_gemm_pipe16_direct(const DcGemmParams* p, int full, int splits, int merged, void* stream);
+
 int64_t dc_gemm_workspace_bytes(void);
 
 int dc_gemm_conv(const DcGemmParams* p, void* stream);
 
 int dc_groupnorm(const uint16_t* x, int ldx, uint16_t* y, int ldy, const float* gamma, const float* beta,
-                 int C, int groups, int n_inst, int rows_per_inst, float eps, int silu,
+                 int C, int groups, int n_inst, int rows_per_inst, float eps, int silu, int out_tiled,
                  float* workspace, void* stream);
 int64_t dc_groupnorm_workspace_bytes(int n_inst, int groups, int rows_per_inst);
 
```

Result: no change. 2.659 frames/s, median of 6 (+0.2%).
